# avikde/robobee3d

Measured on AMD Instinct MI355X. Metric: closed-loop MPC steps/sec (QP+dyn), higher is better.
Workload: dtype f32

## Files before the change

### robobee3d_amd/asmstep.py

```python
import functools
import os
import struct

from . import asmgen, asmtext, symbolic
from .asmgen import (A_D, A_L, A_LO, A_M, A_Q, NLDS, NVZ, S_ALPHA, S_CNT, S_ITERS, S_OMA, S_RHO, S_RINV, S_SIGMA,
                     V_W, V_WZ, V_X, V_Y, V_Z, Emit, f32bits, pk, _sb, _vp)

HERE = os.path.dirname(os.path.abspath(__file__))

PTRS = ["state", "ctrl", "ref", "ws", "out", "stats", "status", "info", "Ib", "gain", "aT0",
        "taskf", "weights", "wl", "wlu", "wlw",
        "done"]
NPTR_RES = 11
INTS = ["stride", "K", "maxIter", "nsub", "plant", "seq"]
TAIL_INTS = ["refstep"]
FLOATS = ["dt", "dtg", "Tmax", "wpr", "wpf", "ws_", "wvr", "wvf", "wds", "wthrust", "wmom",
          "iwpr", "iwpf", "iws", "iwvr", "iwvf", "iwds", "iwthrust", "iwmom",
          "Ib0", "Ib1", "Ib2", "Ibi0", "Ibi1", "Ibi2", "h", "hh", "h6", "taulim", "gpl", "idt", "mbg"]
WNAMES = ["wpr", "wpf", "ws_", "wvr", "wvf", "wds", "wthrust", "wmom"]
WROW = {"ws_": 0, "wds": 1, "wpr": 2, "wpf": 3, "wvr": 4, "wvf": 5, "wthrust": 6, "wmom": 7}
A_W, A_IW = 230, 238
S_PARAM = 4
S_PBLK = 2
S_PTR = {n: 40 + 2 * k for k, n in enumerate(PTRS[:NPTR_RES])}
S_PTR["taskf"], S_PTR["weights"] = 0, 96
S_PTR["wl"], S_PTR["wlu"], S_PTR["wlw"] = 30, 32, 34
S_INT = {"stride": 10, "K": 13, "maxIter": S_ITERS, "nsub": 5, "plant": 39}
S_F = {n: 64 + k for k, n in enumerate(FLOATS)}
assert max(S_F.values()) <= 95
S_STEP, S_SUB, S_RUIZ = 12, 15, 15
S_MBAD, S_MP0 = 62, 14
S_M0, S_M1, S_M2, S_M3 = 30, 32, 34, 36
S_C = {"minscal": 16, "maxscal": 17, "c45": 18, "eps10": 19, "eps": 38, "rho": 6, "rinv": 7, "rmin": 8,
       "rmininv": 9, "infty_ms": 100, "rhotol": 101}
S_TMP = 4
OFF = {}
_o = 0
for _n in PTRS:
    OFF[_n] = _o
    _o += 8
for _n in INTS + FLOATS + TAIL_INTS:
    OFF[_n] = _o
    _o += 4
PARAM_BYTES = _o
HIST_INTS = ["statestep", "outstep", "statusstep", "infostep"]
HIST_OFF = (PARAM_BYTES + 7) // 8 * 8
for _k, _n in enumerate(HIST_INTS):
    OFF[_n] = HIST_OFF + 4 * _k
HIST_BYTES = 4 * len(HIST_INTS)
S_HIST = 32
IMP_OFF = HIST_OFF + HIST_BYTES
assert IMP_OFF % 8 == 0
OFF["imp"], OFF["impstep"] = IMP_OFF, IMP_OFF + 8
IMP_BYTES = 16
S_IMP = 32

VFIRST, VEND = 2, 256
NRING = 6
XV_N, XV_B = 2, 254
NT_PTRS = ("state", "ctrl", "ref", "out", "stats")
A_SPARE, N_SPARE_D = 246, 9


class Pool:

    def __init__(self, e):
        self.e = e
        self.free_ = set(range(VFIRST, VEND))
        self.peak = 0
        self.fixed = set()

    def _take(self, regs):
        for r in regs:
            assert r in self.free_, "v%d is not free" % r
            self.free_.discard(r)
        self.peak = max(self.peak, VEND - VFIRST - len(self.free_))

    def reserve(self, lo, n):
        self._take(range(lo, lo + n))
        return lo

    def get(self):
        cand = sorted(self.free_)
        assert cand, "out of VGPRs"
        for r in cand:
            if (r ^ 1) not in self.free_:
                self._take([r])
                return r
        self._take([cand[0]])
        return cand[0]

    def get2(self):
        for r in sorted(self.free_):
            if r % 2 == 0 and r + 1 in self.free_:
                self._take([r, r + 1])
                return r
        raise AssertionError("out of aligned VGPR pairs")

    def get4(self):
        for r in sorted(self.free_):
            if r % 4 == 0 and all(r + k in self.free_ for k in range(4)):
                self._take([r, r + 1, r + 2, r + 3])
                return r
        raise AssertionError("out of aligned VGPR quads")

    def getn(self, n):
        for r in sorted(self.free_):
            if r % 2 == 0 and all(r + k in self.free_ for k in range(n)):
                self._take(range(r, r + n))
                return r
        raise AssertionError("out of consecutive VGPRs")

    def getn_high(self, n):
# ... 48 lines not shown
    return ("v[%d:%d]" % (base, base + 1), lo_reg % 2, hi_reg % 2)


def PS(sreg):
    if sreg % 2 == 0:
        return ("s[%d:%d]" % (sreg, sreg + 1), 0, 0)
    return ("s[%d:%d]" % (sreg - 1, sreg), 1, 1)


class Struct:
    def __init__(self, N=3, perm=None):
        s = symbolic.analyse(N, perm)
        self.s = s
        self.plan = asmgen.solve_plan(s)
        self.lpos = self.plan[2]
        self.xs, self.zs, self.xinv, self.zinv = asmgen.slot_maps(s)
        nx, nc = s.nx, s.nc
        self.neq = 2 * s.N * symbolic.NY
        self.col_of = [0] * len(s.A_i)
        self.rows = [[] for _ in range(nc)]
        for j in range(nx):
            for p in range(s.A_p[j], s.A_p[j + 1]):
                self.col_of[p] = j
                self.rows[s.A_i[p]].append(p)
        self.unit = {}
        for p, tag in enumerate(s.A_tag):
            if tag[0] == 'c' and abs(tag[1]) == 1.0 and s.A_i[p] not in self.unit:
                self.unit[s.A_i[p]] = (p, self.col_of[p])
        assert len(self.unit) == nc
        used, pairs = set(), []
        for p in range(len(s.A_i)):
            if p in used:
                continue
            i0, j0 = s.A_i[p], self.col_of[p]
            for q_ in range(p + 1, len(s.A_i)):
                if q_ in used:
                    continue
                i1, j1 = s.A_i[q_], self.col_of[q_]
                if (self.zs[i0] ^ 1) == self.zs[i1] and (j0 == j1 or (self.xs[j0] ^ 1) == self.xs[j1]):
                    lo, hi = (p, q_) if self.zs[i0] % 2 == 0 else (q_, p)
                    pairs.append((lo, hi))
                    used.update((p, q_))
                    break
        self.apairs = pairs
        self.asingles = [p for p in range(len(s.A_i)) if p not in used]
        self.apos = [0] * len(s.A_i)
        k = 0
        for (lo, hi) in pairs:
            self.apos[lo], self.apos[hi] = k, k + 1
            k += 2
        for p in self.asingles:
            self.apos[p] = k
            k += 1
        self.na = k
        self.pair_of = {}
        for (lo, hi) in pairs:
            self.pair_of[lo] = self.pair_of[hi] = (lo, hi)
        NYv = symbolic.NY
        self.qnz = list(range(s.N * NYv)) + [s.N * NYv + k_ * NYv + i for k_ in range(s.N) for i in range(3)]
        self.qslot = {}
        for j in range(s.N * NYv):
            self.qslot[j] = self.xs[j]
        base = s.N * NYv
        for k_ in range(s.N):
            for i in range(3):
                self.qslot[s.N * NYv + k_ * NYv + i] = base + 3 * k_ + i
        self.nq = base + 3 * s.N
        self.qzero = frozenset(j for j in range(nx) if j not in self.qslot)
        lnz = set(range(6)) | set(range(3 * 6, 3 * 6 + 6)) | set(range(4 * 6, 4 * 6 + 3)) | {5 * 6 + 2}
        self.lzero = frozenset(i for i in range(self.neq) if i not in lnz) if s.N == 3 else frozenset()

    def weight_of(self, j):
        N, NYv = self.s.N, symbolic.NY
        if j < N * NYv:
            k, i = divmod(j, NYv)
            return ("wpf" if k == N - 1 else "wpr") if i < 3 else "ws_"
        if j < 2 * N * NYv:
            k, i = divmod(j - N * NYv, NYv)
            return ("wvf" if k == N - 1 else "wvr") if i < 3 else "wds"
        return "wthrust" if (j - 2 * N * NYv) % 3 == 0 else "wmom"


class StepGen:
    def __init__(self, N=3, perm=None, quad=False):
        self.st = Struct(N, perm)
        self.s = self.st.s
        self.e = Emit()
        self.pool = Pool(self.e)
        self.lab = 20
        self.quad = quad
        self.nt = () if quad else ("nt",)
        self.homes = asmgen.Homes(NRING, 0 if quad else XV_N, XV_B)

    def label(self):
        self.lab += 1
        return str(self.lab)

    def rcp_nr(self, dst, src, t):
        e = self.e
        e("v_rcp_f32", v(dst), v(src))
        e("s_nop", 0)
        e("v_fma_f32", v(t), "-" + v(src), v(dst), 1.0)
        e("v_fma_f32", v(dst), v(t), v(dst), v(dst))

    def rows_ptr(self, voff, first_row):
        e = self.e
        if first_row == 0:
            e("v_mov_b32", v(voff), "v0")
        else:
            e("s_mul_i32", sg(S_TMP), sg(S_INT["stride"]), first_row)
            e("v_add_u32", v(voff), sg(S_TMP), "v0")

    def load_taskf(self):
        e = self.e
        e("s_lshl_b32", sg(S_TMP), sg(S_STEP), 5)
        e("s_load_dwordx2", sp(S_M0), sp(S_PTR["taskf"]), sg(S_TMP), "offset:0")
        e("s_load_dwordx4", "s[%d:%d]" % (S_M0 + 2, S_M0 + 5), sp(S_PTR["taskf"]), sg(S_TMP), "offset:8")
        e("s_load_dwordx2", sp(S_M0 + 6), sp(S_PTR["taskf"]), sg(S_TMP), "offset:24")
        e("s_waitcnt", "vmcnt(0) lgkmcnt(0)")

    def adv(self, voff):
        self.e("v_add_u32", v(voff), sg(S_INT["stride"]), v(voff))

    def advance_ptr(self, ptr, sstep):
        e, lo = self.e, S_PTR[ptr]
        e("s_add_i32", sg(lo), sg(lo), sg(sstep))
        e("s_cmp_lt_u32", sg(lo), sg(sstep))
        e("s_cselect_b32", sg(sstep), 1, 0)
        e("s_add_i32", sg(lo + 1), sg(lo + 1), sg(sstep))

    def impulse(self, Y0, YS):
        e = self.e
        lab_off = self.label()
        lo, hi, st, oh = S_IMP, S_IMP + 1, S_IMP + 2, S_IMP + 3
        e("s_mov_b32", sg(S_TMP), IMP_OFF)
        e("s_load_dwordx4", "s[%d:%d]" % (S_IMP, S_IMP + 3), sp(S_PBLK), sg(S_TMP))
        e("s_waitcnt", "lgkmcnt(0)")
        e("s_cmp_eq_u64", sp(lo), 0)
        e("s_cbranch_scc1", lab_off + "f")
        e("s_mul_hi_u32", sg(oh), sg(S_STEP), sg(st))
        e("s_mul_i32", sg(st), sg(S_STEP), sg(st))
        e("s_add_i32", sg(hi), sg(hi), sg(oh))
        for i in range(6):
            addend = st if i == 0 else S_INT["stride"]
            lab_nc = self.label()
            e("s_add_i32", sg(lo), sg(lo), sg(addend))
            e("s_cmp_gt_u32", sg(addend), sg(lo))
            e("s_cbranch_scc0", lab_nc + "f")
            e("s_add_i32", sg(hi), sg(hi), 1)
            e("label", lab_nc)
            e("global_load_dword", v(YS + i), "v0", sp(lo))
        e("s_waitcnt", "vmcnt(0)")
        for i in range(6):
            e("v_add_f32", v(Y0 + 12 + i), v(Y0 + 12 + i), v(YS + i))
        e("label", lab_off)

    def load_rows(self, ptr, first_row, regs, voff=None):
        own = voff is None
        if own:
            voff = self.pool.get()
        self.rows_ptr(voff, first_row)
        for k, r in enumerate(regs):
            self.e("global_load_dword", r if isinstance(r, str) else v(r), v(voff), sp(S_PTR[ptr]),
                   *(self.nt if ptr in NT_PTRS or ptr == "ws" else ()))
            if k + 1 < len(regs):
                self.adv(voff)
        if own:
            self.pool.free(voff, kill=False)

    def store_rows(self, ptr, first_row, regs, voff=None):
        own = voff is None
        if own:
            voff = self.pool.get()
        self.rows_ptr(voff, first_row)
        for k, r in enumerate(regs):
            self.e("global_store_dword", v(voff), v(r), sp(S_PTR[ptr]),
                   *(self.nt if ptr in NT_PTRS else ()))
            if k + 1 < len(regs):
                self.adv(voff)
# ... 191 lines not shown
        VP = pool.getn(nx + 1)
        VQ = pool.getn_high(st.nq + st.nq % 2)
        VA = pool.getn(st.na + st.na % 2)
        self.VP, self.VQ, self.VA = VP, VQ, VA
        RP = lambda j: VP + st.xs[j]
        RA = lambda p: VA + st.apos[p]
        RQ = lambda j: VQ + st.qslot[j]
        self.RP, self.RA, self.RQ = RP, RA, RQ
        for j in range(nx):
            e("v_accvgpr_read_b32", v(RP(j)), "a%d" % (A_W + WNAMES.index(st.weight_of(j))))
        e("v_mov_b32", v(VP + nx), 0)
        ydes = RF[0:3] + RF[6:9]
        dpdes = RF[3:6]
        WV = {n: pool.get() for n in ("wpr", "wpf", "ws_", "wvr", "wvf")}
        for n, r in WV.items():
            e("v_accvgpr_read_b32", v(r), "a%d" % (A_W + WNAMES.index(n)))
        for j in st.qnz:
            if j < N * NYv:
                k, i = divmod(j, NYv)
                wname = ("wpf" if k == N - 1 else "wpr") if i < 3 else "ws_"
                e("v_mul_f32", v(RQ(j)), "-" + v(WV[wname]), v(ydes[i]))
            else:
                k, i = divmod(j - N * NYv, NYv)
                e("v_mul_f32", v(RQ(j)), "-" + v(WV["wvf" if k == N - 1 else "wvr"]), v(dpdes[i]))
        if st.nq % 2:
            e("v_mov_b32", v(VQ + st.nq), 0)
        for p, tag in enumerate(s.A_tag):
            if tag[0] == 'c':
                e("v_mov_b32", v(RA(p)), float(tag[1]))
            elif tag[0] == 'dt':
                e("v_mov_b32", v(RA(p)), SF("dt"))
            elif tag[0] == 'T0dt':
                e("v_mov_b32", v(RA(p)), v(dtT0))
            elif tag[0] == 's0':
                e("v_mov_b32", v(RA(p)), v(s0dt[tag[1]]))
            else:
                e("v_mov_b32", v(RA(p)), v(Bdt[tag[1]]))
        if st.na % 2:
            e("v_mov_b32", v(VA + st.na), 0)
        pool.free(dtT0, *s0dt, *Bdt, t)
        pool.free(*ST)
        pool.free(*RF)
        pool.free(*WV.values())
        pool.free_range(LS, 20)
        self.ruiz_quad() if self.quad else self.ruiz()
        self.recover_and_bounds()
        self.factor()

    def maxabs(self, dst, regs, acc_in=False):
        e = self.e
        regs = list(regs)
        if not acc_in:
            if len(regs) == 1:
                e("v_and_b32", v(dst), 0x7fffffff, v(regs[0]))
                return
            if len(regs) == 2:
                e("v_max_f32", v(dst), "|%s|" % v(regs[0]), "|%s|" % v(regs[1]))
                return
            e("v_max3_f32", v(dst), "|%s|" % v(regs[0]), "|%s|" % v(regs[1]), "|%s|" % v(regs[2]))
            regs = regs[3:]
        while len(regs) >= 2:
            e("v_max3_f32", v(dst), v(dst), "|%s|" % v(regs[0]), "|%s|" % v(regs[1]))
            regs = regs[2:]
        if regs:
            e("v_max_f32", v(dst), v(dst), "|%s|" % v(regs[0]))

    def limit(self, regs, rsq):
        e = self.e
        regs = list(regs)
        prev = None
        for r in regs + [None]:
            if r is not None:
                e("v_cmp_lt_f32", "vcc", sg(S_C["minscal"]), v(r))
            if prev is not None:
                e("v_min_f32", v(prev), sg(S_C["maxscal"]), v(prev))
            if r is not None:
                e("v_cndmask_b32", v(r), 1.0, v(r), "vcc")
            prev = r
        if rsq:
            for r in regs:
                e("v_rsq_f32", v(r), v(r))
            e("s_nop", 0)

    def ruiz(self):
        e, pool, st, s = self.e, self.pool, self.st, self.s
        nx, nc = s.nx, s.nc
        RP, RA, RQ = self.RP, self.RA, self.RQ
        VE = pool.getn(nc + 1)
        self.VE = VE
        RE = lambda i: VE + st.zs[i]
        self.RE = RE
        cs = pool.get()
        self.cs = cs
        e("v_mov_b32", v(cs), 1.0)
        e("v_mov_b32", v(VE + nc), 0)
        e("s_mov_b32", sg(S_RUIZ), 10)
        top = self.label()
        e("label", top)
        for i in range(nc):
            self.maxabs(RE(i), [RA(p) for p in st.rows[i]])
        self.limit([RE(i) for i in range(nc)], rsq=True)
        colpairs = [(st.xinv[2 * k], st.xinv[2 * k + 1]) for k in range(nx // 2)]
        if nx % 2:
            colpairs.append((st.xinv[nx - 1], None))
        CH = 3
        for c0 in range(0, len(colpairs), CH):
            chunk = colpairs[c0:c0 + CH]
            T = [pool.get2() for _ in chunk]
            for (j0, j1), t2 in zip(chunk, T):
                for h, j in enumerate((j0, j1)):
                    if j is None:
                        e("v_mov_b32", v(t2 + 1), 1.0)
                        continue
                    self.maxabs(t2 + h, [RP(j)] + [RA(p) for p in range(s.A_p[j], s.A_p[j + 1])])
            self.limit([t2 + h for (j0, j1), t2 in zip(chunk, T) for h, j in enumerate((j0, j1)) if j is not None], rsq=True)
            for (j0, j1), t2 in zip(chunk, T):
                cols = [j for j in (j0, j1) if j is not None]
                tcol = {j0: t2}
                if j1 is not None:
                    tcol[j1] = t2 + 1
                ents = [p for j in cols for p in range(s.A_p[j], s.A_p[j + 1])]
                pairs = sorted({st.pair_of[p] for p in ents if p in st.pair_of})
                singles = [p for p in ents if p not in st.pair_of]
                for (lo, hi) in pairs:
                    assert st.col_of[lo] in tcol and st.col_of[hi] in tcol
                for (lo, hi) in pairs:
                    pk(e, "v_pk_mul_f32", RA(lo), [P2(RA(lo)), PSEL(RE(s.A_i[lo]), RE(s.A_i[hi]))])
                for p in singles:
                    e("v_mul_f32", v(RA(p)), v(RA(p)), v(RE(s.A_i[p])))
                if j1 is not None:
                    pk(e, "v_pk_mul_f32", RP(j0), [P2(RP(j0)), P2(t2)])
                else:
                    e("v_mul_f32", v(RP(j0)), v(RP(j0)), v(t2))
                qj = [j for j in cols if j in st.qslot]
                if len(qj) == 2 and RQ(qj[0]) % 2 == 0 and RQ(qj[1]) == RQ(qj[0]) + 1:
                    pk(e, "v_pk_mul_f32", RQ(qj[0]), [P2(RQ(qj[0])), P2(t2)])
                else:
                    for j in qj:
                        e("v_mul_f32", v(RQ(j)), v(RQ(j)), v(tcol[j]))
                for (lo, hi) in pairs:
                    pk(e, "v_pk_mul_f32", RA(lo), [P2(RA(lo)), PSEL(tcol[st.col_of[lo]], tcol[st.col_of[hi]])])
                for p in singles:
                    e("v_mul_f32", v(RA(p)), v(RA(p)), v(tcol[st.col_of[p]]))
                if j1 is not None:
                    pk(e, "v_pk_mul_f32", RP(j0), [P2(RP(j0)), P2(t2)])
                else:
                    e("v_mul_f32", v(RP(j0)), v(RP(j0)), v(t2))
            for t2 in T:
                pool.free(t2, t2 + 1)
        acc = pool.get2()
        VP, VQ = self.VP, self.VQ
        pk(e, "v_pk_add_f32", acc, [P2(VP), P2(VP + 2)])
        for k in range(4, nx + 1, 2):
            pk(e, "v_pk_add_f32", acc, [P2(acc), P2(VP + k)])
        qn, ct, t = pool.get(), pool.get(), pool.get()
        self.maxabs(qn, [VQ + k for k in range(st.nq)])
        e("v_add_f32", v(acc), v(acc), v(acc + 1))
        e("v_mul_f32", v(acc), sg(S_C["c45"]), v(acc))
        self.limit([qn], rsq=False)
        e("v_max_f32", v(acc), v(acc), v(qn))
        self.limit([acc], rsq=False)
        self.rcp_nr(ct, acc, t)
        for k in range(0, nx + 1, 2):
            pk(e, "v_pk_mul_f32", VP + k, [P2(VP + k), PB(ct)])
        for k in range(0, st.nq + st.nq % 2, 2):
            pk(e, "v_pk_mul_f32", VQ + k, [P2(VQ + k), PB(ct)])
        e("v_mul_f32", v(cs), v(cs), v(ct))
        pool.free(acc, acc + 1, qn, ct, t)
        e("s_sub_i32", sg(S_RUIZ), sg(S_RUIZ), 1)
        e("s_cmp_gt_i32", sg(S_RUIZ), 0)
        e("s_cbranch_scc1", top + "b")


    def ruiz_quad(self):
        from . import asmquad, asmquad64
        e, pool, st, s = self.e, self.pool, self.st, self.s
        nx, nc = s.nx, s.nc
        RP, RA, RQ = self.RP, self.RA, self.RQ
        VE = pool.getn(nc + 1)
        self.VE = VE
        self.RE = lambda i: VE + st.zs[i]
        cs = pool.get()
        self.cs = cs
        e("v_mov_b32", v(cs), 1.0)
        e("v_mov_b32", v(VE + nc), 0)
        qp = asmquad.QuadPlan(st)
        rp = asmquad64.RuizQuadPlan(s, qp)
        hostA = {key: RA(d[min(d)]) for key, d in rp.slots.items()}
        colmem = {}
        for j in range(nx):
            ln, C = qp.xhome[j]
            colmem.setdefault(C, {})[ln] = j
        hostP = {C: RP(m[min(m)]) for C, m in colmem.items()}
        hostQ = {C: RQ(min(jj for jj in m.values() if jj in st.qslot)) for C, m in colmem.items() if any(jj in st.qslot for jj in m.values())}
        for C, m in colmem.items():
            if C in hostQ:
                assert all(jj in st.qslot for jj in m.values())
        dead = [RA(p) for key, d in rp.slots.items() for ln, p in d.items() if RA(p) != hostA[key]] + \
               [RP(j) for C, m in colmem.items() for j in m.values() if RP(j) != hostP[C]]
        dead = sorted(set(dead))
        ET = [dead.pop() for _ in range(13)]
        DT = [dead.pop() for _ in range(15)]
        t, m7, acc, qn, ct, tt = (dead.pop() for _ in range(6))
        masks = (asmquad.S_L0, asmquad.S_L1, asmquad.S_L2)
        S_L3 = 98
        keep = sorted(set(range(self.VP, self.VP + nx + 1)) | set(range(self.VQ, self.VQ + st.nq + st.nq % 2)) |
                      set(range(self.VA, self.VA + st.na + st.na % 2)) | {cs, VE + nc})
        e("quad_begin", "ruiz")
        e("s_mov_b64", sp(asmquad.S_EXEC), "exec")
        for ln, m in enumerate(masks + (S_L3,)):
            e("s_mov_b32", sg(m), 0x11111111 << ln)
            e("s_mov_b32", sg(m + 1), 0x11111111 << ln)
            e("s_and_b64", sp(m), sp(m), sp(asmquad.S_EXEC))
        for ln in (1, 2):
            e("s_mov_b64", "exec", sp(masks[ln]))
            for key, d in rp.slots.items():
                if ln in d and RA(d[ln]) != hostA[key]:
                    e("v_mov_b32", v(hostA[key]), v(RA(d[ln])))
                elif ln not in d:
                    e("v_mov_b32", v(hostA[key]), 0)
            for C, m in colmem.items():
                if ln in m:
                    if RP(m[ln]) != hostP[C]:
                        e("v_mov_b32", v(hostP[C]), v(RP(m[ln])))
                    if C in hostQ and RQ(m[ln]) != hostQ[C]:
                        e("v_mov_b32", v(hostQ[C]), v(RQ(m[ln])))
        for key, d in rp.slots.items():
            if 0 not in d:
                e("s_mov_b64", "exec", sp(masks[0]))
                e("v_mov_b32", v(hostA[key]), 0)
                e("s_mov_b64", "exec", sp(S_L3))
                e("v_mov_b32", v(hostA[key]), 0)
        e("s_mov_b64", "exec", sp(asmquad.S_EXEC))
        e("s_nop", 4)
        e("s_mov_b32", sg(S_RUIZ), 10)
        top = self.label()
        e("label", top)
        byrow, bycol = {}, {}
        for key in sorted(rp.slots):
            byrow.setdefault(key[0], []).append(key)
            bycol.setdefault(key[1], []).append(key)
        for R in range(13):
            self.maxabs(ET[R], [hostA[k] for k in byrow[R]])
        self.limit(ET, rsq=True)
        for C in range(15):
            own = [k for k in bycol.get(C, []) if rp.kind[k] == "own"]
            self.maxabs(DT[C], [hostP[C]] + [hostA[k] for k in own])
            for k in [k for k in bycol.get(C, []) if rp.kind[k] != "own"]:
                r = hostA[k]
                e("v_max_f32_dpp", v(m7), "|%s|" % v(r), "|%s|" % v(r), asmquad.qperm(asmquad64.ROT1))
                e("v_max_f32_dpp", v(m7), "|%s|" % v(r), v(m7), asmquad.qperm(asmquad64.ROT2))
                e("s_mov_b64", "exec", sp(masks[rp.kind[k]]))
                e("v_max_f32", v(DT[C]), v(DT[C]), v(m7))
                e("s_mov_b64", "exec", sp(asmquad.S_EXEC))
                e("s_nop", 4)
# ... 1051 lines not shown
            e("s_mov_b64", "exec", sp(m))
            e("v_mov_b32", v(Q0), v(Y0 + r))
            e("v_mov_b32", v(Q0 + 1), v(Y0 + 12 + r))
            for c in range(3):
                e("v_mov_b32", v(Q0 + 2 + c), v(Y0 + 3 + r + 3 * c))
            if r == 2:
                e("v_mov_b32", v(G), SF("gpl"))
        e("s_mov_b64", "exec", sp(S_EX))
        for i in range(3):
            e("v_mov_b32", v(Q0 + 5 + i), v(Y0 + 15 + i))
        e("s_nop", 4)

        def vf(src, dst):
            p_, v_, r0, r1, r2, wx, wy, wz = (src + k for k in range(8))
            e("v_mov_b32", v(dst), v(v_))
            e("v_mul_f32", v(dst + 1), v(Th), v(r2))
            e("v_sub_f32", v(dst + 1), v(dst + 1), v(G))
            e("v_mul_f32", v(a), v(r2), v(wy))
            e("v_fma_f32", v(dst + 2), v(r1), v(wz), "-" + v(a))
            e("v_mul_f32", v(b), v(r0), v(wz))
            e("v_fma_f32", v(dst + 3), v(r2), v(wx), "-" + v(b))
            e("v_mul_f32", v(a), v(r1), v(wx))
            e("v_fma_f32", v(dst + 4), v(r0), v(wy), "-" + v(a))
            hx, hy, hz = dst + 5, dst + 6, dst + 7
            e("v_mul_f32", v(hx), v(Ib[0]), v(wx))
            e("v_mul_f32", v(hy), v(Ib[1]), v(wy))
            e("v_mul_f32", v(hz), v(Ib[2]), v(wz))
            e("v_mul_f32", v(a), v(wz), v(hy))
            e("v_fma_f32", v(a), v(wy), v(hz), "-" + v(a))
            e("v_mul_f32", v(b), v(wx), v(hz))
            e("v_fma_f32", v(b), v(wz), v(hx), "-" + v(b))
            e("v_mul_f32", v(hz), v(wy), v(hx))
            e("v_fma_f32", v(hz), v(wx), v(hy), "-" + v(hz))
            e("v_sub_f32", v(a), v(u1), v(a))
            e("v_mul_f32", v(dst + 5), v(a), v(Ibi[0]))
            e("v_sub_f32", v(b), v(u2), v(b))
            e("v_mul_f32", v(dst + 6), v(b), v(Ibi[1]))
            e("v_mul_f32", v(dst + 7), "-" + v(hz), v(Ibi[2]))
        e("s_mov_b32", sg(S_SUB), sg(S_INT["nsub"]))
        top = self.label()
        e("label", top)
        vf(Q0, QA)
        for k in range(0, 8, 2):
            pk(e, "v_pk_fma_f32", QS + k, [PS(S_F["hh"]), P2(QA + k), P2(Q0 + k)])
        vf(QS, QK)
        for k in range(0, 8, 2):
            pk(e, "v_pk_fma_f32", QA + k, [PB(two), P2(QK + k), P2(QA + k)])
            pk(e, "v_pk_fma_f32", QS + k, [PS(S_F["hh"]), P2(QK + k), P2(Q0 + k)])
        vf(QS, QK)
        for k in range(0, 8, 2):
            pk(e, "v_pk_fma_f32", QA + k, [PB(two), P2(QK + k), P2(QA + k)])
            pk(e, "v_pk_fma_f32", QS + k, [PS(S_F["h"]), P2(QK + k), P2(Q0 + k)])
        vf(QS, QK)
        for k in range(0, 8, 2):
            pk(e, "v_pk_add_f32", QA + k, [P2(QA + k), P2(QK + k)])
        for k in range(0, 8, 2):
            pk(e, "v_pk_fma_f32", Q0 + k, [PS(S_F["h6"]), P2(QA + k), P2(Q0 + k)])
        e("s_nop", 1)
        for r in range(3):
            e("v_mov_b32_dpp", v(PA + r), v(Q0), asmquad.qperm([r] * 4))
        e("s_nop", 1)
        for r in range(3):
            e("v_fmac_f32", v(serr), v(PA + r), v(PA + r))
        e("v_add_f32", v(seff), v(seff), v(einc))
        e("s_sub_i32", sg(S_SUB), sg(S_SUB), 1)
        e("s_cmp_gt_i32", sg(S_SUB), 0)
        e("s_cbranch_scc1", top + "b")
        e("s_nop", 1)
        for r in range(3):
            e("v_mov_b32_dpp", v(Y0 + r), v(Q0), asmquad.qperm([r] * 4))
            e("v_mov_b32_dpp", v(Y0 + 12 + r), v(Q0 + 1), asmquad.qperm([r] * 4))
            for c in range(3):
                e("v_mov_b32_dpp", v(Y0 + 3 + r + 3 * c), v(Q0 + 2 + c), asmquad.qperm([r] * 4))
        for i in range(3):
            e("v_mov_b32", v(Y0 + 15 + i), v(Q0 + 5 + i))
        e("s_nop", 1)
        e("quad_end", tuple(keep))

    def program(self):
        e = self.e
        self.prologue()
        top = self.label()
        e("label", top)
        self.phase_a()
        self.admm()
        self.phase_c()
        e("s_load_dword", sg(S_TMP), sp(S_PBLK), OFF["refstep"])
        e("s_load_dwordx4", "s[%d:%d]" % (S_HIST, S_HIST + 3), sp(S_PBLK), HIST_OFF)
        e("s_waitcnt", "lgkmcnt(0)")
        e("s_add_u32", sg(S_PTR["ref"]), sg(S_PTR["ref"]), sg(S_TMP))
        e("s_addc_u32", sg(S_PTR["ref"] + 1), sg(S_PTR["ref"] + 1), 0)
        for n in ("out", "status", "info"):
            self.advance_ptr(n, S_HIST + HIST_INTS.index(n + "step"))
        e("s_add_i32", sg(S_STEP), sg(S_STEP), 1)
        e("s_cmp_lt_i32", sg(S_STEP), sg(S_INT["K"]))
        e("s_cbranch_scc1", top + "b")
        e("s_waitcnt", "vmcnt(0) lgkmcnt(0)")
        lab = self.label()
        e("s_load_dwordx2", sp(S_M0), sp(S_PBLK), OFF["done"])
        e("s_load_dword", sg(S_M1), sp(S_PBLK), OFF["seq"])
        e("s_waitcnt", "lgkmcnt(0)")
        e("s_cmp_eq_u64", sp(S_M0), 0)
        e("s_cbranch_scc1", lab + "f")
        e("buffer_wbl2", "sc0 sc1")
        e("s_waitcnt", "vmcnt(0)")
        a, b = self.pool.get(), self.pool.get()
        e("v_mov_b32", v(a), 0)
        e("v_mov_b32", v(b), sg(S_M1))
        e("global_store_dword", v(a), v(b), sp(S_M0), "sc0 sc1")
        e("s_waitcnt", "vmcnt(0)")
        self.pool.free(a, b)
        e("label", lab)
        return e.ins


fmt = functools.partial(asmtext.fmt, hex_ints=asmtext.HEX_ABOVE_64)


PSEUDO = ("kill", "quad_begin", "quad_end")


def write(path=None, N=3, perm=None, quad=False):
    path = path or os.path.join(HERE, "csrc", "umpc_step_asm_quad.h" if quad else "umpc_step_asm.h")
    g = StepGen(N, perm, quad=quad)
    ins = [t for t in g.program() if t[0] not in PSEUDO]
    if quad:
        head = ["// GENERATED by robobee3d_amd/asmstep.py (quad=True) + asmquad.py -- do not edit.", asmgen.switch_banner(),
               "// The all-assembly fp32 step kernel body, ONE ROBOT PER LANE QUAD (16 robots per wavefront): %d instructions."
               % len(ins),
               "// Every lane of a quad gets the same v0 (= 4 * robot) and its own LDS slice; include umpc_step_asm.h first (StepParams).",
               "#pragma once"]
    else:
        head = ["// GENERATED by robobee3d_amd/asmstep.py -- do not edit.", asmgen.switch_banner(),
               "// The all-assembly fp32 step kernel body: %d instructions (K closed-loop steps of one wavefront)." % len(ins),
               "#pragma once", "#include <stddef.h>", "#include <stdint.h>", "namespace umpcasm {",
               "// parameter block read by the kernel with s_load (byte offsets are part of the generated code)",
               "struct StepParams {"]
        for n in PTRS:
            head.append("  const void *%s;" % n)
        for n in INTS:
            head.append("  int32_t %s;" % n)
        for n in FLOATS:
            head.append("  float %s;" % n)
        for n in TAIL_INTS:
            head.append("  int32_t %s;" % n)
        head += ["};", "static_assert(sizeof(StepParams) == %d, \"StepParams layout\");" % ((PARAM_BYTES + 7) // 8 * 8),
                "// step history (umpcBatchSetHistory): bytes the state / out / status / info pointers advance per closed-loop step,",
                "// read by the stream at byte %d of the kernarg segment: the kernels take ONE StepArgs as their first argument" % HIST_OFF,
                "struct StepHist {"] + ["  int32_t %s;" % n for n in HIST_INTS] + ["};",
                "// velocity impulses (umpcBatchSetImpulses): slice `cursor` of the table [steps][6][B] (null: none) and the bytes per slice,",
                "// read by the stream at byte %d of the kernarg segment" % IMP_OFF,
                "struct StepImp {", "  const void *imp;", "  int32_t impstep;", "  int32_t pad_;", "};",
                "struct StepArgs {", "  StepParams p;", "  StepHist h;", "  StepImp i;", "};",
                "static_assert(offsetof(StepArgs, h) == %d && sizeof(StepHist) == %d, \"StepHist layout\");" % (HIST_OFF, HIST_BYTES),
                "static_assert(offsetof(StepArgs, i) == %d && sizeof(StepImp) == %d && offsetof(StepImp, impstep) == 8, \"StepImp layout\");" % (IMP_OFF, IMP_BYTES),
                "constexpr int STEP_LDS_BYTES_PER_LANE = %d;" % (NLDS * 4), "}  // namespace umpcasm",
                "// inputs: v0 = 4 * robot, v1 = lane LDS address, s[4:5] = &StepParams (kernarg)"]
    asmtext.write_if_changed(path, asmtext.asm_block(
        head, "UMPC_STEP_ASM%s(voff, ldsaddr, params)" % ("_QUAD" if quad else ""), ins,
        '"{v0}"(voff), "{v1}"(ldsaddr), "{s[4:5]}"(params)',
        asmtext.clobbers(range(2, 256), range(256), range(4, 102)), fmt))
    return path, len(ins)


_KEEP_V = {0, 1} | set(range(V_W, V_Z)) | set(range(V_Z + 2 * 3 * symbolic.NY, V_Z + 40))
QUAD = {None: None}


def _quad():
    from . import isasim
    if QUAD[None] is None:
        QUAD.update({None: isasim.Quad(v=_KEEP_V, dead_v=set(range(256)) - _KEEP_V, a=range(A_LO, 256), dead_a=range(A_LO)),
                     "ruiz": isasim.Quad(a=range(256)), "plant": isasim.Quad(a=range(256))})
    return QUAD


FLAT = ("taskf", "wl")
STRIDE = 4096
PBASE = 0x00007E0080000000


def simulate(ins, arrays, ints, floats, max_exec=3000000, ptr_xform=None):
    import numpy as np
    from . import isasim
    base_of = {n: 0x00007F0080000000 + (k << 36) for k, n in enumerate(PTRS + ["impulse"])}
    ptr_xform = ptr_xform or (lambda a: a)
    blob = bytearray(IMP_OFF + IMP_BYTES)
    for n in PTRS:
        struct.pack_into("<Q", blob, OFF[n], ptr_xform(base_of[n]) if arrays.get(n) is not None else 0)
    allints = dict(ints, stride=STRIDE)
    allints.setdefault("seq", 0)
    allints.setdefault("refstep", 0)
    for n in HIST_INTS:
        allints.setdefault(n, 0)
    for n in INTS + TAIL_INTS + HIST_INTS:
        struct.pack_into("<i", blob, OFF[n], int(allints[n]))
    for n in FLOATS:
        struct.pack_into("<f", blob, OFF[n], float(floats[n]))
    allints.setdefault("impstep", 6 * STRIDE if arrays.get("impulse") is not None else 0)
    struct.pack_into("<Q", blob, OFF["imp"], ptr_xform(base_of["impulse"]) if arrays.get("impulse") is not None else 0)
    struct.pack_into("<i", blob, OFF["impstep"], int(allints["impstep"]))
    regions = [(PBASE, 4, np.frombuffer(bytes(blob), np.uint32))] + \
        [(base_of[n], 4 if n in FLAT else STRIDE, arrays[n]) for n in PTRS + ["impulse"] if arrays.get(n) is not None]
    m = isasim.Machine(ins, regions=regions, sgpr={S_PARAM: PBASE & 0xFFFFFFFF, S_PARAM + 1: PBASE >> 32}, vgpr={0: 0},
                       lds=np.zeros((1, NLDS), np.uint32), max_exec=max_exec, quad=_quad())
    isasim.run(m)
    simulate.last_quad_sections = {("admm" if k is None else k): n for k, n in m.sections.items()}
    simulate.last_quad_instructions = sum(m.sections.values())
    return m.nexec


if __name__ == "__main__":
    p, n = write()
    print("wrote", p, n, "instructions")


def host_floats(dt=5.0, g=9.81e-3, TtoWmax=2.0, ws=1e1, wds=1e3, wpr=1.0, wpf=5.0, wvr=1e3, wvf=2e3, wthrust=1e-1, wmom=1e-2,
                Ib=(3333.0, 3333.0, 1000.0), dtsim=0.2, taulim=100.0, mb=100.0):
    import numpy as np
    f = np.float32
    one = f(1.0)
    w = dict(wpr=f(wpr), wpf=f(wpf), ws_=f(ws), wvr=f(wvr), wvf=f(wvf), wds=f(wds), wthrust=f(wthrust), wmom=f(wmom))
    d = dict(dt=f(dt), dtg=f(f(dt) * f(g)), Tmax=f(f(TtoWmax) * f(g)), **w)
    for k, val in w.items():
        d["i" + k.rstrip("_")] = f(one / val)
    for i in range(3):
        d["Ib%d" % i] = f(Ib[i])
        d["Ibi%d" % i] = f(one / f(Ib[i]))
    d.update(h=f(dtsim), hh=f(f(0.5) * f(dtsim)), h6=f(f(dtsim) / f(6.0)), taulim=f(taulim), gpl=f(9.81e-3), idt=f(one / f(dt)),
             mbg=f(f(mb) * f(g)))
    assert set(d) == set(FLOATS), set(FLOATS) ^ set(d)
    return {k: float(val) for k, val in d.items()}
```

### robobee3d_amd/csrc/umpc_step_asm.h

```cpp
#pragma once
#include <stddef.h>
#include <stdint.h>
namespace umpcasm {
struct StepParams {
  const void *state;
  const void *ctrl;
  const void *ref;
  const void *ws;
  const void *out;
  const void *stats;
  const void *status;
  const void *info;
  const void *Ib;
  const void *gain;
  const void *aT0;
  const void *taskf;
  const void *weights;
  const void *wl;
  const void *wlu;
  const void *wlw;
  const void *done;
  int32_t stride;
  int32_t K;
  int32_t maxIter;
// ... 13 lines not shown
  float wmom;
  float iwpr;
  float iwpf;
  float iws;
  float iwvr;
  float iwvf;
  float iwds;
  float iwthrust;
  float iwmom;
  float Ib0;
  float Ib1;
  float Ib2;
  float Ibi0;
  float Ibi1;
  float Ibi2;
  float h;
  float hh;
  float h6;
  float taulim;
  float gpl;
  float idt;
  float mbg;
  int32_t refstep;
};
static_assert(sizeof(StepParams) == 296, "StepParams layout");
struct StepHist {
  int32_t statestep;
  int32_t outstep;
  int32_t statusstep;
  int32_t infostep;
};
struct StepImp {
  const void *imp;
  int32_t impstep;
  int32_t pad_;
};
struct StepArgs {
  StepParams p;
  StepHist h;
  StepImp i;
};
static_assert(offsetof(StepArgs, h) == 296 && sizeof(StepHist) == 16, "StepHist layout");
static_assert(offsetof(StepArgs, i) == 312 && sizeof(StepImp) == 16 && offsetof(StepImp, impstep) == 8, "StepImp layout");
constexpr int STEP_LDS_BYTES_PER_LANE = 640;
}
#define UMPC_STEP_ASM(voff, ldsaddr, params) asm volatile( \
  "s_mov_b64 s[2:3], s[4:5]\n" \
  "s_load_dwordx16 s[40:55], s[2:3], 0x0\n" \
  "s_load_dwordx4 s[56:59], s[2:3], 0x40\n" \
  "s_load_dwordx2 s[60:61], s[2:3], 0x50\n" \
  "s_load_dwordx2 s[0:1], s[2:3], 0x58\n" \
  "s_load_dwordx2 s[96:97], s[2:3], 0x60\n" \
  "s_load_dwordx16 s[64:79], s[2:3], 0xa0\n" \
  "s_load_dwordx16 s[80:95], s[2:3], 0xe0\n" \
  "s_load_dword s10, s[2:3], 0x88\n" \
  "s_load_dword s13, s[2:3], 0x8c\n" \
  "s_load_dword s11, s[2:3], 0x90\n" \
  "s_load_dword s5, s[2:3], 0x94\n" \
  "s_load_dword s39, s[2:3], 0x98\n" \
  "s_mov_b32 s20, 0x3fcccccd\n" \
  "s_mov_b32 s21, 0x3fcccccd\n" \
  "s_mov_b32 s22, 0xbf19999a\n" \
  "s_mov_b32 s23, 0xbf19999a\n" \
  "s_mov_b32 s24, 0x358637bd\n" \
  "s_mov_b32 s25, 0x358637bd\n" \
  "s_mov_b32 s26, 0x3c23d70a\n" \
  "s_mov_b32 s27, 0x3c23d70a\n" \
  "s_mov_b32 s28, 0x42c80000\n" \
  "s_mov_b32 s29, 0x42c80000\n" \
  "s_mov_b32 s16, 0x38d1b717\n" \
  "s_mov_b32 s17, 0x461c4000\n" \
  "s_mov_b32 s18, 0x3cb60b61\n" \
  "s_mov_b32 s38, 0x38d1b717\n" \
  "s_mov_b32 s19, 0x3a83126e\n" \
  "s_mov_b32 s6, 0x3dcccccd\n" \
  "s_mov_b32 s7, 0x41200000\n" \
  "s_mov_b32 s8, 0x358637bd\n" \
  "s_mov_b32 s9, 0x49742400\n" \
  "s_mov_b32 s100, 0x6aa56fa6\n" \
  "s_mov_b32 s101, 0x38d1b717\n" \
  "s_waitcnt lgkmcnt(0)\n" \
  "s_mov_b32 s12, 0\n" \
  "21:\n" \
  "v_mov_b32 v33, v0\n" \
  "global_load_dword v2, v33, s[40:41] nt\n" \
  "v_add_u32 v33, s10, v33\n" \
  "global_load_dword v3, v33, s[40:41] nt\n" \
  "v_add_u32 v33, s10, v33\n" \
  "global_load_dword v4, v33, s[40:41] nt\n" \
  "v_add_u32 v33, s10, v33\n" \
  "global_load_dword v5, v33, s[40:41] nt\n" \
  "v_add_u32 v33, s10, v33\n" \
  "global_load_dword v6, v33, s[40:41] nt\n" \
  "v_add_u32 v33, s10, v33\n" \
  "global_load_dword v7, v33, s[40:41] nt\n" \
  "v_add_u32 v33, s10, v33\n" \
  "global_load_dword v8, v33, s[40:41] nt\n" \
  "v_add_u32 v33, s10, v33\n" \
  "global_load_dword v9, v33, s[40:41] nt\n" \
  "v_add_u32 v33, s10, v33\n" \
  "global_load_dword v10, v33, s[40:41] nt\n" \
  "v_add_u32 v33, s10, v33\n" \
  "global_load_dword v11, v33, s[40:41] nt\n" \
  "v_add_u32 v33, s10, v33\n" \
  "global_load_dword v12, v33, s[40:41] nt\n" \
  "v_add_u32 v33, s10, v33\n" \
  "global_load_dword v13, v33, s[40:41] nt\n" \
  "v_add_u32 v33, s10, v33\n" \
  "global_load_dword v14, v33, s[40:41] nt\n" \
  "v_add_u32 v33, s10, v33\n" \
  "global_load_dword v15, v33, s[40:41] nt\n" \
  "v_add_u32 v33, s10, v33\n" \
  "global_load_dword v16, v33, s[40:41] nt\n" \
  "v_add_u32 v33, s10, v33\n" \
  "global_load_dword v17, v33, s[40:41] nt\n" \
  "v_add_u32 v33, s10, v33\n" \
  "global_load_dword v18, v33, s[40:41] nt\n" \
  "v_add_u32 v33, s10, v33\n" \
  "global_load_dword v19, v33, s[40:41] nt\n" \
  "v_mov_b32 v33, v0\n" \
  "global_load_dword v20, v33, s[44:45] nt\n" \
  "v_add_u32 v33, s10, v33\n" \
  "global_load_dword v21, v33, s[44:45] nt\n" \
  "v_add_u32 v33, s10, v33\n" \
  "global_load_dword v22, v33, s[44:45] nt\n" \
  "v_add_u32 v33, s10, v33\n" \
  "global_load_dword v23, v33, s[44:45] nt\n" \
  "v_add_u32 v33, s10, v33\n" \
  "global_load_dword v24, v33, s[44:45] nt\n" \
  "v_add_u32 v33, s10, v33\n" \
  "global_load_dword v25, v33, s[44:45] nt\n" \
  "v_add_u32 v33, s10, v33\n" \
  "global_load_dword v26, v33, s[44:45] nt\n" \
  "v_add_u32 v33, s10, v33\n" \
  "global_load_dword v27, v33, s[44:45] nt\n" \
  "v_add_u32 v33, s10, v33\n" \
  "global_load_dword v28, v33, s[44:45] nt\n" \
  "s_mul_i32 s4, s10, 0x7b\n" \
  "v_add_u32 v33, s4, v0\n" \
  "global_load_dword v29, v33, s[42:43] nt\n" \
  "v_add_u32 v33, s10, v33\n" \
  "global_load_dword v30, v33, s[42:43] nt\n" \
  "v_add_u32 v33, s10, v33\n" \
  "global_load_dword v31, v33, s[42:43] nt\n" \
  "v_add_u32 v33, s10, v33\n" \
  "global_load_dword v32, v33, s[42:43] nt\n" \
  "s_cmp_eq_u64 s[96:97], 0\n" \
  "s_cbranch_scc1 22f\n" \
  "v_mov_b32 v33, v0\n" \
  "global_load_dword v36, v33, s[96:97]\n" \
  "v_add_u32 v33, s10, v33\n" \
  "global_load_dword v39, v33, s[96:97]\n" \
  "v_add_u32 v33, s10, v33\n" \
  "global_load_dword v34, v33, s[96:97]\n" \
  "v_add_u32 v33, s10, v33\n" \
  "global_load_dword v35, v33, s[96:97]\n" \
  "v_add_u32 v33, s10, v33\n" \
  "global_load_dword v37, v33, s[96:97]\n" \
  "v_add_u32 v33, s10, v33\n" \
  "global_load_dword v38, v33, s[96:97]\n" \
  "v_add_u32 v33, s10, v33\n" \
  "global_load_dword v40, v33, s[96:97]\n" \
  "v_add_u32 v33, s10, v33\n" \
  "global_load_dword v41, v33, s[96:97]\n" \
  "s_waitcnt vmcnt(0)\n" \
  "v_rcp_f32 v42, v34\n" \
// ... 356 lines not shown
  "v_mov_b32 v145, -1.0\n" \
  "v_mov_b32 v148, s64\n" \
  "v_mov_b32 v150, -1.0\n" \
  "v_mov_b32 v152, 1.0\n" \
  "v_mov_b32 v149, s64\n" \
  "v_mov_b32 v151, -1.0\n" \
  "v_mov_b32 v153, 1.0\n" \
  "v_mov_b32 v154, s64\n" \
  "v_mov_b32 v156, -1.0\n" \
  "v_mov_b32 v158, 1.0\n" \
  "v_mov_b32 v160, s64\n" \
  "v_mov_b32 v162, -1.0\n" \
  "v_mov_b32 v164, 1.0\n" \
  "v_mov_b32 v161, s64\n" \
  "v_mov_b32 v163, -1.0\n" \
  "v_mov_b32 v165, 1.0\n" \
  "v_mov_b32 v155, s64\n" \
  "v_mov_b32 v157, -1.0\n" \
  "v_mov_b32 v159, 1.0\n" \
  "v_mov_b32 v166, s64\n" \
  "v_mov_b32 v168, -1.0\n" \
  "v_mov_b32 v170, 1.0\n" \
  "v_mov_b32 v167, s64\n" \
  "v_mov_b32 v169, -1.0\n" \
  "v_mov_b32 v171, 1.0\n" \
  "v_mov_b32 v172, s64\n" \
  "v_mov_b32 v174, -1.0\n" \
  "v_mov_b32 v176, 1.0\n" \
  "v_mov_b32 v178, s64\n" \
  "v_mov_b32 v180, -1.0\n" \
  "v_mov_b32 v182, 1.0\n" \
  "v_mov_b32 v179, s64\n" \
  "v_mov_b32 v181, -1.0\n" \
  "v_mov_b32 v183, 1.0\n" \
  "v_mov_b32 v173, s64\n" \
  "v_mov_b32 v175, -1.0\n" \
  "v_mov_b32 v177, 1.0\n" \
  "v_mov_b32 v184, s64\n" \
  "v_mov_b32 v186, -1.0\n" \
  "v_mov_b32 v185, s64\n" \
  "v_mov_b32 v187, -1.0\n" \
  "v_mov_b32 v188, s64\n" \
  "v_mov_b32 v190, -1.0\n" \
  "v_mov_b32 v192, s64\n" \
  "v_mov_b32 v194, -1.0\n" \
  "v_mov_b32 v193, s64\n" \
  "v_mov_b32 v195, -1.0\n" \
  "v_mov_b32 v189, s64\n" \
  "v_mov_b32 v191, -1.0\n" \
  "v_mov_b32 v196, v45\n" \
  "v_mov_b32 v197, v30\n" \
  "v_mov_b32 v198, v31\n" \
  "v_mov_b32 v219, 1.0\n" \
  "v_mov_b32 v200, v34\n" \
  "v_mov_b32 v201, v35\n" \
  "v_mov_b32 v199, v66\n" \
  "v_mov_b32 v202, v67\n" \
  "v_mov_b32 v203, v68\n" \
  "v_mov_b32 v220, v69\n" \
  "v_mov_b32 v204, v45\n" \
  "v_mov_b32 v205, v30\n" \
  "v_mov_b32 v221, v31\n" \
  "v_mov_b32 v222, 1.0\n" \
  "v_mov_b32 v206, v34\n" \
  "v_mov_b32 v207, v35\n" \
  "v_mov_b32 v223, v66\n" \
  "v_mov_b32 v208, v67\n" \
  "v_mov_b32 v209, v68\n" \
  "v_mov_b32 v224, v69\n" \
  "v_mov_b32 v210, v45\n" \
  "v_mov_b32 v211, v30\n" \
  "v_mov_b32 v212, v31\n" \
  "v_mov_b32 v225, 1.0\n" \
  "v_mov_b32 v214, v34\n" \
  "v_mov_b32 v215, v35\n" \
  "v_mov_b32 v213, v66\n" \
  "v_mov_b32 v216, v67\n" \
  "v_mov_b32 v217, v68\n" \
  "v_mov_b32 v226, v69\n" \
  "v_mov_b32 v227, 0\n" \
  "v_mov_b32 v42, 1.0\n" \
  "v_mov_b32 v41, 0\n" \
  "s_mov_b32 s15, 10\n" \
  "28:\n" \
  "v_max_f32 v2, |v116|, |v148|\n" \
  "v_max_f32 v3, |v117|, |v149|\n" \
  "v_max_f32 v4, |v120|, |v154|\n" \
  "v_max_f32 v6, |v124|, |v160|\n" \
  "v_max_f32 v7, |v125|, |v161|\n" \
  "v_max_f32 v5, |v121|, |v155|\n" \
  "v_max3_f32 v8, |v118|, |v130|, |v166|\n" \
  "v_max3_f32 v9, |v119|, |v131|, |v167|\n" \
  "v_max3_f32 v10, |v122|, |v134|, |v172|\n" \
  "v_max3_f32 v12, |v126|, |v138|, |v178|\n" \
  "v_max3_f32 v13, |v127|, |v139|, |v179|\n" \
  "v_max3_f32 v11, |v123|, |v135|, |v173|\n" \
  "v_max3_f32 v14, |v132|, |v142|, |v184|\n" \
  "v_max3_f32 v15, |v133|, |v143|, |v185|\n" \
  "v_max3_f32 v16, |v136|, |v144|, |v188|\n" \
  "v_max3_f32 v18, |v140|, |v146|, |v192|\n" \
  "v_max3_f32 v19, |v141|, |v147|, |v193|\n" \
  "v_max3_f32 v17, |v137|, |v145|, |v189|\n" \
  "v_max_f32 v20, |v150|, |v196|\n" \
  "v_max_f32 v21, |v151|, |v197|\n" \
  "v_max_f32 v22, |v156|, |v198|\n" \
  "v_max3_f32 v24, |v162|, |v200|, |v202|\n" \
  "v_max3_f32 v25, |v163|, |v201|, |v203|\n" \
  "v_max3_f32 v23, |v157|, |v199|, |v220|\n" \
  "v_max3_f32 v26, |v152|, |v168|, |v204|\n" \
  "v_max3_f32 v27, |v153|, |v169|, |v205|\n" \
  "v_max3_f32 v28, |v158|, |v174|, |v221|\n" \
  "v_max3_f32 v30, |v164|, |v180|, |v206|\n" \
  "v_max_f32 v30, v30, |v208|\n" \
  "v_max3_f32 v31, |v165|, |v181|, |v207|\n" \
  "v_max_f32 v31, v31, |v209|\n" \
  "v_max3_f32 v29, |v159|, |v175|, |v223|\n" \
  "v_max_f32 v29, v29, |v224|\n" \
  "v_max3_f32 v32, |v128|, |v170|, |v186|\n" \
  "v_max_f32 v32, v32, |v210|\n" \
  "v_max3_f32 v33, |v129|, |v171|, |v187|\n" \
  "v_max_f32 v33, v33, |v211|\n" \
  "v_max3_f32 v34, |v218|, |v176|, |v190|\n" \
  "v_max_f32 v34, v34, |v212|\n" \
  "v_max3_f32 v36, |v182|, |v194|, |v214|\n" \
  "v_max_f32 v36, v36, |v216|\n" \
  "v_max3_f32 v37, |v183|, |v195|, |v215|\n" \
  "v_max_f32 v37, v37, |v217|\n" \
  "v_max3_f32 v35, |v177|, |v191|, |v213|\n" \
  "v_max_f32 v35, v35, |v226|\n" \
  "v_and_b32 v38, 0x7fffffff, v219\n" \
  "v_and_b32 v39, 0x7fffffff, v222\n" \
  "v_and_b32 v40, 0x7fffffff, v225\n" \
  "v_cmp_lt_f32 vcc, s16, v2\n" \
  "v_cndmask_b32 v2, 1.0, v2, vcc\n" \
  "v_cmp_lt_f32 vcc, s16, v3\n" \
  "v_min_f32 v2, s17, v2\n" \
  "v_cndmask_b32 v3, 1.0, v3, vcc\n" \
  "v_cmp_lt_f32 vcc, s16, v4\n" \
  "v_min_f32 v3, s17, v3\n" \
  "v_cndmask_b32 v4, 1.0, v4, vcc\n" \
  "v_cmp_lt_f32 vcc, s16, v6\n" \
  "v_min_f32 v4, s17, v4\n" \
  "v_cndmask_b32 v6, 1.0, v6, vcc\n" \
  "v_cmp_lt_f32 vcc, s16, v7\n" \
  "v_min_f32 v6, s17, v6\n" \
  "v_cndmask_b32 v7, 1.0, v7, vcc\n" \
  "v_cmp_lt_f32 vcc, s16, v5\n" \
  "v_min_f32 v7, s17, v7\n" \
  "v_cndmask_b32 v5, 1.0, v5, vcc\n" \
  "v_cmp_lt_f32 vcc, s16, v8\n" \
  "v_min_f32 v5, s17, v5\n" \
  "v_cndmask_b32 v8, 1.0, v8, vcc\n" \
  "v_cmp_lt_f32 vcc, s16, v9\n" \
  "v_min_f32 v8, s17, v8\n" \
  "v_cndmask_b32 v9, 1.0, v9, vcc\n" \
  "v_cmp_lt_f32 vcc, s16, v10\n" \
  "v_min_f32 v9, s17, v9\n" \
  "v_cndmask_b32 v10, 1.0, v10, vcc\n" \
  "v_cmp_lt_f32 vcc, s16, v12\n" \
  "v_min_f32 v10, s17, v10\n" \
  "v_cndmask_b32 v12, 1.0, v12, vcc\n" \
  "v_cmp_lt_f32 vcc, s16, v13\n" \
  "v_min_f32 v12, s17, v12\n" \
  "v_cndmask_b32 v13, 1.0, v13, vcc\n" \
  "v_cmp_lt_f32 vcc, s16, v11\n" \
  "v_min_f32 v13, s17, v13\n" \
// ... 567 lines not shown
  "v_pk_add_f32 v[44:45], v[44:45], v[80:81] op_sel:[0,0] op_sel_hi:[1,1] neg_lo:[0,0] neg_hi:[0,0]\n" \
  "v_pk_add_f32 v[44:45], v[44:45], v[82:83] op_sel:[0,0] op_sel_hi:[1,1] neg_lo:[0,0] neg_hi:[0,0]\n" \
  "v_pk_add_f32 v[44:45], v[44:45], v[84:85] op_sel:[0,0] op_sel_hi:[1,1] neg_lo:[0,0] neg_hi:[0,0]\n" \
  "v_pk_add_f32 v[44:45], v[44:45], v[86:87] op_sel:[0,0] op_sel_hi:[1,1] neg_lo:[0,0] neg_hi:[0,0]\n" \
  "v_pk_add_f32 v[44:45], v[44:45], v[88:89] op_sel:[0,0] op_sel_hi:[1,1] neg_lo:[0,0] neg_hi:[0,0]\n" \
  "v_pk_add_f32 v[44:45], v[44:45], v[90:91] op_sel:[0,0] op_sel_hi:[1,1] neg_lo:[0,0] neg_hi:[0,0]\n" \
  "v_pk_add_f32 v[44:45], v[44:45], v[92:93] op_sel:[0,0] op_sel_hi:[1,1] neg_lo:[0,0] neg_hi:[0,0]\n" \
  "v_pk_add_f32 v[44:45], v[44:45], v[94:95] op_sel:[0,0] op_sel_hi:[1,1] neg_lo:[0,0] neg_hi:[0,0]\n" \
  "v_pk_add_f32 v[44:45], v[44:45], v[96:97] op_sel:[0,0] op_sel_hi:[1,1] neg_lo:[0,0] neg_hi:[0,0]\n" \
  "v_pk_add_f32 v[44:45], v[44:45], v[98:99] op_sel:[0,0] op_sel_hi:[1,1] neg_lo:[0,0] neg_hi:[0,0]\n" \
  "v_pk_add_f32 v[44:45], v[44:45], v[100:101] op_sel:[0,0] op_sel_hi:[1,1] neg_lo:[0,0] neg_hi:[0,0]\n" \
  "v_pk_add_f32 v[44:45], v[44:45], v[102:103] op_sel:[0,0] op_sel_hi:[1,1] neg_lo:[0,0] neg_hi:[0,0]\n" \
  "v_pk_add_f32 v[44:45], v[44:45], v[104:105] op_sel:[0,0] op_sel_hi:[1,1] neg_lo:[0,0] neg_hi:[0,0]\n" \
  "v_pk_add_f32 v[44:45], v[44:45], v[106:107] op_sel:[0,0] op_sel_hi:[1,1] neg_lo:[0,0] neg_hi:[0,0]\n" \
  "v_pk_add_f32 v[44:45], v[44:45], v[108:109] op_sel:[0,0] op_sel_hi:[1,1] neg_lo:[0,0] neg_hi:[0,0]\n" \
  "v_pk_add_f32 v[44:45], v[44:45], v[110:111] op_sel:[0,0] op_sel_hi:[1,1] neg_lo:[0,0] neg_hi:[0,0]\n" \
  "v_pk_add_f32 v[44:45], v[44:45], v[112:113] op_sel:[0,0] op_sel_hi:[1,1] neg_lo:[0,0] neg_hi:[0,0]\n" \
  "v_pk_add_f32 v[44:45], v[44:45], v[114:115] op_sel:[0,0] op_sel_hi:[1,1] neg_lo:[0,0] neg_hi:[0,0]\n" \
  "v_max3_f32 v43, |v228|, |v229|, |v230|\n" \
  "v_max3_f32 v43, v43, |v231|, |v232|\n" \
  "v_max3_f32 v43, v43, |v233|, |v234|\n" \
  "v_max3_f32 v43, v43, |v235|, |v236|\n" \
  "v_max3_f32 v43, v43, |v237|, |v238|\n" \
  "v_max3_f32 v43, v43, |v239|, |v240|\n" \
  "v_max3_f32 v43, v43, |v241|, |v242|\n" \
  "v_max3_f32 v43, v43, |v243|, |v244|\n" \
  "v_max3_f32 v43, v43, |v245|, |v246|\n" \
  "v_max3_f32 v43, v43, |v247|, |v248|\n" \
  "v_max3_f32 v43, v43, |v249|, |v250|\n" \
  "v_max3_f32 v43, v43, |v251|, |v252|\n" \
  "v_max3_f32 v43, v43, |v253|, |v254|\n" \
  "v_add_f32 v44, v44, v45\n" \
  "v_mul_f32 v44, s18, v44\n" \
  "v_cmp_lt_f32 vcc, s16, v43\n" \
  "v_cndmask_b32 v43, 1.0, v43, vcc\n" \
  "v_min_f32 v43, s17, v43\n" \
  "v_max_f32 v44, v44, v43\n" \
  "v_cmp_lt_f32 vcc, s16, v44\n" \
  "v_cndmask_b32 v44, 1.0, v44, vcc\n" \
  "v_min_f32 v44, s17, v44\n" \
  "v_rcp_f32 v46, v44\n" \
  "s_nop 0\n" \
  "v_fma_f32 v47, -v44, v46, 1.0\n" \
  "v_fma_f32 v46, v47, v46, v46\n" \
  "v_pk_mul_f32 v[70:71], v[70:71], v[46:47] op_sel:[0,0] op_sel_hi:[1,0] neg_lo:[0,0] neg_hi:[0,0]\n" \
  "v_pk_mul_f32 v[72:73], v[72:73], v[46:47] op_sel:[0,0] op_sel_hi:[1,0] neg_lo:[0,0] neg_hi:[0,0]\n" \
  "v_pk_mul_f32 v[74:75], v[74:75], v[46:47] op_sel:[0,0] op_sel_hi:[1,0] neg_lo:[0,0] neg_hi:[0,0]\n" \
  "v_pk_mul_f32 v[76:77], v[76:77], v[46:47] op_sel:[0,0] op_sel_hi:[1,0] neg_lo:[0,0] neg_hi:[0,0]\n" \
  "v_pk_mul_f32 v[78:79], v[78:79], v[46:47] op_sel:[0,0] op_sel_hi:[1,0] neg_lo:[0,0] neg_hi:[0,0]\n" \
  "v_pk_mul_f32 v[80:81], v[80:81], v[46:47] op_sel:[0,0] op_sel_hi:[1,0] neg_lo:[0,0] neg_hi:[0,0]\n" \
  "v_pk_mul_f32 v[82:83], v[82:83], v[46:47] op_sel:[0,0] op_sel_hi:[1,0] neg_lo:[0,0] neg_hi:[0,0]\n" \
  "v_pk_mul_f32 v[84:85], v[84:85], v[46:47] op_sel:[0,0] op_sel_hi:[1,0] neg_lo:[0,0] neg_hi:[0,0]\n" \
  "v_pk_mul_f32 v[86:87], v[86:87], v[46:47] op_sel:[0,0] op_sel_hi:[1,0] neg_lo:[0,0] neg_hi:[0,0]\n" \
  "v_pk_mul_f32 v[88:89], v[88:89], v[46:47] op_sel:[0,0] op_sel_hi:[1,0] neg_lo:[0,0] neg_hi:[0,0]\n" \
  "v_pk_mul_f32 v[90:91], v[90:91], v[46:47] op_sel:[0,0] op_sel_hi:[1,0] neg_lo:[0,0] neg_hi:[0,0]\n" \
  "v_pk_mul_f32 v[92:93], v[92:93], v[46:47] op_sel:[0,0] op_sel_hi:[1,0] neg_lo:[0,0] neg_hi:[0,0]\n" \
  "v_pk_mul_f32 v[94:95], v[94:95], v[46:47] op_sel:[0,0] op_sel_hi:[1,0] neg_lo:[0,0] neg_hi:[0,0]\n" \
  "v_pk_mul_f32 v[96:97], v[96:97], v[46:47] op_sel:[0,0] op_sel_hi:[1,0] neg_lo:[0,0] neg_hi:[0,0]\n" \
  "v_pk_mul_f32 v[98:99], v[98:99], v[46:47] op_sel:[0,0] op_sel_hi:[1,0] neg_lo:[0,0] neg_hi:[0,0]\n" \
  "v_pk_mul_f32 v[100:101], v[100:101], v[46:47] op_sel:[0,0] op_sel_hi:[1,0] neg_lo:[0,0] neg_hi:[0,0]\n" \
  "v_pk_mul_f32 v[102:103], v[102:103], v[46:47] op_sel:[0,0] op_sel_hi:[1,0] neg_lo:[0,0] neg_hi:[0,0]\n" \
  "v_pk_mul_f32 v[104:105], v[104:105], v[46:47] op_sel:[0,0] op_sel_hi:[1,0] neg_lo:[0,0] neg_hi:[0,0]\n" \
  "v_pk_mul_f32 v[106:107], v[106:107], v[46:47] op_sel:[0,0] op_sel_hi:[1,0] neg_lo:[0,0] neg_hi:[0,0]\n" \
  "v_pk_mul_f32 v[108:109], v[108:109], v[46:47] op_sel:[0,0] op_sel_hi:[1,0] neg_lo:[0,0] neg_hi:[0,0]\n" \
  "v_pk_mul_f32 v[110:111], v[110:111], v[46:47] op_sel:[0,0] op_sel_hi:[1,0] neg_lo:[0,0] neg_hi:[0,0]\n" \
  "v_pk_mul_f32 v[112:113], v[112:113], v[46:47] op_sel:[0,0] op_sel_hi:[1,0] neg_lo:[0,0] neg_hi:[0,0]\n" \
  "v_pk_mul_f32 v[114:115], v[114:115], v[46:47] op_sel:[0,0] op_sel_hi:[1,0] neg_lo:[0,0] neg_hi:[0,0]\n" \
  "v_pk_mul_f32 v[228:229], v[228:229], v[46:47] op_sel:[0,0] op_sel_hi:[1,0] neg_lo:[0,0] neg_hi:[0,0]\n" \
  "v_pk_mul_f32 v[230:231], v[230:231], v[46:47] op_sel:[0,0] op_sel_hi:[1,0] neg_lo:[0,0] neg_hi:[0,0]\n" \
  "v_pk_mul_f32 v[232:233], v[232:233], v[46:47] op_sel:[0,0] op_sel_hi:[1,0] neg_lo:[0,0] neg_hi:[0,0]\n" \
  "v_pk_mul_f32 v[234:235], v[234:235], v[46:47] op_sel:[0,0] op_sel_hi:[1,0] neg_lo:[0,0] neg_hi:[0,0]\n" \
  "v_pk_mul_f32 v[236:237], v[236:237], v[46:47] op_sel:[0,0] op_sel_hi:[1,0] neg_lo:[0,0] neg_hi:[0,0]\n" \
  "v_pk_mul_f32 v[238:239], v[238:239], v[46:47] op_sel:[0,0] op_sel_hi:[1,0] neg_lo:[0,0] neg_hi:[0,0]\n" \
  "v_pk_mul_f32 v[240:241], v[240:241], v[46:47] op_sel:[0,0] op_sel_hi:[1,0] neg_lo:[0,0] neg_hi:[0,0]\n" \
  "v_pk_mul_f32 v[242:243], v[242:243], v[46:47] op_sel:[0,0] op_sel_hi:[1,0] neg_lo:[0,0] neg_hi:[0,0]\n" \
  "v_pk_mul_f32 v[244:245], v[244:245], v[46:47] op_sel:[0,0] op_sel_hi:[1,0] neg_lo:[0,0] neg_hi:[0,0]\n" \
  "v_pk_mul_f32 v[246:247], v[246:247], v[46:47] op_sel:[0,0] op_sel_hi:[1,0] neg_lo:[0,0] neg_hi:[0,0]\n" \
  "v_pk_mul_f32 v[248:249], v[248:249], v[46:47] op_sel:[0,0] op_sel_hi:[1,0] neg_lo:[0,0] neg_hi:[0,0]\n" \
  "v_pk_mul_f32 v[250:251], v[250:251], v[46:47] op_sel:[0,0] op_sel_hi:[1,0] neg_lo:[0,0] neg_hi:[0,0]\n" \
  "v_pk_mul_f32 v[252:253], v[252:253], v[46:47] op_sel:[0,0] op_sel_hi:[1,0] neg_lo:[0,0] neg_hi:[0,0]\n" \
  "v_pk_mul_f32 v[254:255], v[254:255], v[46:47] op_sel:[0,0] op_sel_hi:[1,0] neg_lo:[0,0] neg_hi:[0,0]\n" \
  "v_mul_f32 v42, v42, v46\n" \
  "s_sub_i32 s15, s15, 1\n" \
  "s_cmp_gt_i32 s15, 0\n" \
  "s_cbranch_scc1 28b\n" \
  "v_rcp_f32 v43, v42\n" \
  "s_nop 0\n" \
  "v_fma_f32 v44, -v42, v43, 1.0\n" \
  "v_fma_f32 v43, v44, v43, v43\n" \
  "s_mul_i32 s4, s10, 9\n" \
  "v_add_u32 v47, s4, v0\n" \
  "v_accvgpr_read_b32 v48, a238\n" \
  "v_accvgpr_read_b32 v49, a239\n" \
  "v_accvgpr_read_b32 v50, a240\n" \
  "v_accvgpr_read_b32 v51, a241\n" \
  "v_accvgpr_read_b32 v52, a242\n" \
  "v_accvgpr_read_b32 v53, a243\n" \
  "v_accvgpr_read_b32 v54, a244\n" \
  "v_accvgpr_read_b32 v55, a245\n" \
  "v_mul_f32 v45, v70, v43\n" \
  "v_mul_f32 v45, v48, v45\n" \
  "v_sqrt_f32 v45, v45\n" \
  "s_nop 0\n" \
  "v_accvgpr_write_b32 a246, v45\n" \
  "v_rcp_f32 v46, v45\n" \
  "s_nop 0\n" \
  "v_mul_f32 v2, |v116|, v46\n" \
  "v_mul_f32 v8, |v118|, v46\n" \
  "v_mul_f32 v45, v71, v43\n" \
  "v_mul_f32 v45, v48, v45\n" \
  "v_sqrt_f32 v45, v45\n" \
  "s_nop 0\n" \
  "v_accvgpr_write_b32 a247, v45\n" \
  "v_rcp_f32 v46, v45\n" \
  "s_nop 0\n" \
  "v_mul_f32 v3, |v117|, v46\n" \
  "v_mul_f32 v9, |v119|, v46\n" \
  "v_mul_f32 v45, v72, v43\n" \
  "v_mul_f32 v45, v48, v45\n" \
  "v_sqrt_f32 v45, v45\n" \
  "s_nop 0\n" \
  "v_accvgpr_write_b32 a248, v45\n" \
  "v_rcp_f32 v46, v45\n" \
  "s_nop 0\n" \
  "v_mul_f32 v4, |v120|, v46\n" \
  "v_mul_f32 v10, |v122|, v46\n" \
  "v_mul_f32 v45, v74, v43\n" \
  "v_mul_f32 v45, v50, v45\n" \
  "v_sqrt_f32 v45, v45\n" \
  "s_nop 0\n" \
  "v_accvgpr_write_b32 a249, v45\n" \
  "v_rcp_f32 v46, v45\n" \
  "s_nop 0\n" \
  "v_mul_f32 v6, |v124|, v46\n" \
  "v_mul_f32 v12, |v126|, v46\n" \
  "v_mul_f32 v45, v75, v43\n" \
  "v_mul_f32 v45, v50, v45\n" \
  "v_sqrt_f32 v45, v45\n" \
  "s_nop 0\n" \
  "v_accvgpr_write_b32 a250, v45\n" \
  "v_rcp_f32 v46, v45\n" \
  "s_nop 0\n" \
  "v_mul_f32 v7, |v125|, v46\n" \
  "v_mul_f32 v13, |v127|, v46\n" \
  "v_mul_f32 v45, v73, v43\n" \
  "v_mul_f32 v45, v50, v45\n" \
  "v_sqrt_f32 v45, v45\n" \
  "s_nop 0\n" \
  "v_accvgpr_write_b32 a251, v45\n" \
  "v_rcp_f32 v46, v45\n" \
  "s_nop 0\n" \
  "v_mul_f32 v5, |v121|, v46\n" \
  "v_mul_f32 v11, |v123|, v46\n" \
  "v_mul_f32 v45, v76, v43\n" \
  "v_mul_f32 v45, v48, v45\n" \
  "v_sqrt_f32 v45, v45\n" \
  "s_nop 0\n" \
  "v_accvgpr_write_b32 a252, v45\n" \
  "v_rcp_f32 v46, v45\n" \
  "s_nop 0\n" \
  "v_mul_f32 v14, |v132|, v46\n" \
  "v_mul_f32 v45, v77, v43\n" \
  "v_mul_f32 v45, v48, v45\n" \
  "v_sqrt_f32 v45, v45\n" \
  "s_nop 0\n" \
  "v_accvgpr_write_b32 a253, v45\n" \
  "v_rcp_f32 v46, v45\n" \
  "s_nop 0\n" \
// ... 7783 lines not shown
```

### robobee3d_amd/isasim.py

```python
import functools
import re
from fractions import Fraction

import numpy as np

f32, f64, u32, u64 = np.float32, np.float64, np.uint32, np.uint64
POISON = 0x7ff8dead
VCC = 106
LANE_LDS_VGPR = 1


class AddressFault(Exception):
    """A simulated global access outside every array handed to the interpreter (on the GPU: a memory access fault)."""


class Quad:

    def __init__(self, v=(), a=(), lds=(), dead_v=(), dead_a=(), dead_lds=()):
        self.v, self.a, self.lds = list(v), list(a), list(lds)
        self.dead_v, self.dead_a, self.dead_lds = list(dead_v), list(dead_a), list(dead_lds)


_REG = re.compile(r"([vas])(\d+)$|([vas])\[(\d+):(\d+)\]$")

# ... 10 lines not shown
    x = x[1:-1] if ab else x
    if x == "vcc":
        return ("s", VCC, 2, neg, ab)
    if x == "exec":
        return ("exec", 0, 2, neg, ab)
    mm = _REG.match(x)
    if mm is None:
        raise ValueError("operand %r" % x)
    if mm.group(1):
        return (mm.group(1), int(mm.group(2)), 1, neg, ab)
    return (mm.group(3), int(mm.group(4)), int(mm.group(5)) - int(mm.group(4)) + 1, neg, ab)


@functools.lru_cache(maxsize=None)
def _regs(x):
    if not isinstance(x, str):
        return frozenset()
    x = x.lstrip("-").strip("|")
    if x == "vcc":
        return frozenset({("s", VCC), ("s", VCC + 1)})
    mm = _REG.match(x)
    if mm is None:
        return frozenset()
    if mm.group(1):
        return frozenset({(mm.group(1), int(mm.group(2)))})
    return frozenset((mm.group(3), r) for r in range(int(mm.group(4)), int(mm.group(5)) + 1))


def _srcs(t, k):
    x, d = t[k], t[-1]
    if isinstance(x, dict):
        return frozenset()
    if not isinstance(d, dict) or k < 2:
        return _regs(x)
    kind, lo = _decode(x)[:2]
    q = k - 2
    sels = (d["op_sel"][q],) if t[0] == "v_pk_mov_b32" else (d["op_sel"][q], d["op_sel_hi"][q])
    return frozenset((kind, lo + h) for h in sels)


def _fmax(a, b):
    return np.where(b != b, a, np.where(a != a, b, np.where(b > a, b, a)))


def _fmin(a, b):
    return np.where(b != b, a, np.where(a != a, b, np.where(b < a, b, a)))


def _imm(t, k):
    for x in t[k:]:
        if isinstance(x, int):
            return x
        if isinstance(x, str) and x.startswith("offset:"):
            return int(x[7:])
    return 0


_CMP = {"lt": np.less, "le": np.less_equal, "gt": np.greater, "ge": np.greater_equal, "eq": np.equal,
        "nlt": lambda a, b: ~(a < b), "neq": lambda a, b: ~(a == b), "ne": np.not_equal, "u": lambda a, b: (a != a) | (b != b)}
_WAITABLE = ("ds_read", "global_load", "s_load")
_T1_READ = ("ds_write", "ds_min", "global_store", "s_cmp", "s_cbranch", "s_branch", "v_fmac")


class Machine:
    def __init__(self, ins, lanes=1, regions=(), sgpr=None, vgpr=None, lds=None, max_exec=3000000, quad=None, log=None,
                 V=None, A=None):
        self.ins, self.lanes = ins, lanes
        self.V = np.full((lanes, 256), POISON, u32) if V is None else V
        self.A = np.full((lanes, 256), POISON, u32) if A is None else A
        self.S = [0] * 128
        for r, val in (sgpr or {}).items():
            self.S[r] = val & 0xFFFFFFFF
        if V is None:
            for r, val in (vgpr or {}).items():
                self.V[:, r] = val
            self.V[:, LANE_LDS_VGPR] = 16 * np.arange(lanes)
        self.lds = np.zeros((1, 0), u32) if lds is None else lds
        self.regions = [(b, st, arr, arr.view(u32).reshape(-1), arr.itemsize) for b, st, arr in regions]
        self.set_exec(np.ones(lanes, bool))
        self.scc = 0
        self.max_exec, self.quad, self.log = max_exec, quad or {}, log
        self.nexec = 0
        self.sections = {}
        self.pend = {"vmcnt": [], "lgkmcnt": []}
        self.labels = {}
        for k, t in enumerate(ins):
            if t[0] == "label":
                self.labels.setdefault(t[1], []).append(k)
        self._use, self._rw = {}, {}
        self.dead = set()
        self.src_word, self.src_phase, self.phase = {}, {}, 0

    def set_exec(self, bits):
        self.exec, self.full, self.any = bits, bool(bits.all()), bool(bits.any())

    def mask64(self, bits):
        return sum(1 << ln for ln in range(self.lanes) if bits[ln])

    def lanes_of(self, m):
        return np.array([(m >> ln) & 1 for ln in range(self.lanes)], bool)

    def s32(self, x):
        k, lo = _decode(x)[:2]
        return lo & 0xFFFFFFFF if k == "i" else self.S[lo]

    def s64(self, x):
        k, lo = _decode(x)[:2]
        if k == "i":
            return lo & 0xFFFFFFFFFFFFFFFF
        if k == "exec":
            return self.mask64(self.exec)
        return self.S[lo] | (self.S[lo + 1] << 32)

    def set64(self, x, val):
        k, lo = _decode(x)[:2]
        if k == "exec":
            self.set_exec(self.lanes_of(val))
        else:
            self.S[lo], self.S[lo + 1] = val & 0xFFFFFFFF, (val >> 32) & 0xFFFFFFFF

    def bits(self, x, dpp=None):
        k, lo, _, neg, ab = _decode(x)
        if k == "f":
            b = np.full(self.lanes, np.array(lo, f32).view(u32), u32)
        elif k == "i":
            b = np.full(self.lanes, lo & 0xFFFFFFFF, u32)
        elif k == "s":
            b = np.full(self.lanes, self.S[lo], u32)
        else:
            b = (self.V if k == "v" else self.A)[:, lo].copy()
            if dpp is not None:
                qp = [int(c) for c in dpp[dpp.index("[") + 1:dpp.index("]")].split(",")][:self.lanes]
                for ln in range(self.lanes):
                    if self.exec[ln] and not self.exec[qp[ln]]:
                        raise AssertionError("DPP read of a masked-off lane: %r" % (dpp,))
                b = b[qp]
        if ab:
            b = b & u32(0x7FFFFFFF)
        return b ^ u32(0x80000000) if neg else b

    def f(self, x, dpp=None):
        return self.bits(x, dpp).view(f32)

    def d(self, x):
        k, lo, _, neg, ab = _decode(x)
        if k == "f":
            val = np.full(self.lanes, lo, f64)
        else:
            if k == "s":
                b = np.full(self.lanes, self.S[lo] | (self.S[lo + 1] << 32), u64)
            else:
                R = self.V if k == "v" else self.A
                b = R[:, lo].astype(u64) | (R[:, lo + 1].astype(u64) << u64(32))
            val = b.view(f64)
        if ab:
            val = np.abs(val)
        return -val if neg else val

    def write(self, x, b, lo_off=0):
        k, lo = _decode(x)[:2]
        R = self.V if k == "v" else self.A
        if self.full:
            R[:, lo + lo_off] = b
        else:
            R[self.exec, lo + lo_off] = np.asarray(b, u32)[self.exec]

# ... 28 lines not shown
        w = (byte // 1024) * 4 + (byte % 16) // 4
        if w >= self.lds.shape[1]:
            raise AddressFault("%r touches LDS byte 0x%x, outside the lane's slice" % (self.ins[self.pc], byte))
        return ln, w

    def active(self):
        return [ln for ln in range(self.lanes) if self.exec[ln]]

    def uses(self, pc):
        u = self._use.get(pc)
        if u is None:
            t = self.ins[pc]
            u = self._use[pc] = set().union(*[_regs(x) for x in t[1:] if not isinstance(x, dict)])
        return u

    def wait(self, t):
        for part in " ".join(str(x) for x in t[1:]).split():
            name, val = part[:-1].split("(")
            del self.pend[name][:max(0, len(self.pend[name]) - int(val))]

    def track(self, pc, m):
        used = self.uses(pc)
        for q in self.pend.values():
            for dst in q:
                assert not (dst & used), ("register used before its load was waited for", pc, self.ins[pc], sorted(dst & used))
        if m.startswith(_WAITABLE):
            (self.pend["vmcnt"] if m.startswith("global") else self.pend["lgkmcnt"]).append(_regs(self.ins[pc][1]))
        elif m.startswith("ds_"):
            self.pend["lgkmcnt"].append(set())
        elif m.startswith("global_"):
            self.pend["vmcnt"].append(set())
        if self.dead:
            rw = self._rw.get(pc)
            if rw is None:
                t = self.ins[pc]
                dst = frozenset() if m.startswith(_T1_READ) else _regs(t[1])
                rw = self._rw[pc] = (set().union(*[_srcs(t, k) for k in range(2 if dst else 1, len(t))]), dst)
            assert not (rw[0] & self.dead), ("register read after its kill", pc, self.ins[pc], sorted(rw[0] & self.dead))
            self.dead -= rw[1]
        if self.log is not None:
            self.log_reads(pc, m, used)

    def log_reads(self, pc, m, used):
        if m.startswith("ds_read"):
            return
        t = self.ins[pc]
        wr_only = _regs(t[1]) if m in ("global_load_dword", "v_mov_b32", "v_accvgpr_read_b32") else set()
        for r in wr_only:
            self.src_word.pop(r, None)
        for r in used - wr_only:
            if r in self.src_word:
                if self.src_phase[r] == self.phase:
                    self.log["r"].add(self.src_word[r])
                else:
                    self.log["late"].add((self.src_phase[r], self.src_word[r]))

    def branch(self, target):
        lab, d = target[:-1], target[-1]
        cands = self.labels[lab]
        self.pc = min(c for c in cands if c > self.pc) if d == "f" else max(c for c in cands if c < self.pc)

    def run(self, pc=0):
        ins = self.ins
        self.pc = pc
        with np.errstate(all="ignore"):
            while self.pc < len(ins):
                t = ins[self.pc]
                m = t[0]
                if m == "label":
                    self.pc += 1
                    continue
                if m == "kill":
                    self.V[:, _decode(t[1])[1]] = POISON
                    self.dead |= _regs(t[1])
                    self.pc += 1
                    continue
                if m == "quad_begin":
                    self.run_quad(t)
                    continue
                if m == "quad_end":
                    return
                self.nexec += 1
                assert self.nexec < self.max_exec, "runaway program"
                if m == "s_waitcnt":
                    self.wait(t)
                elif m == "s_barrier":
                    assert not self.pend["lgkmcnt"], ("s_barrier with LDS operations in flight: another wave may not see them", self.pc)
                    yield self.pc
                    self.phase += 1
                else:
                    op = OPS.get(m)
                    if op is None:
                        raise ValueError("unknown instruction %r" % (t,))
                    self.track(self.pc, m)
                    if self.any or m in SALU or m == "v_readfirstlane_b32":
                        op(self, t)
                self.pc += 1

    def run_quad(self, t):
        assert self.lanes == 1 and self.exec.all()
        name = t[1] if len(t) > 1 else None
        spec = self.quad[name]
        q = Machine(self.ins, 4, lds=np.tile(self.lds, (4, 1)), max_exec=self.max_exec,
                    V=np.tile(self.V, (4, 1)), A=np.tile(self.A, (4, 1)))
        q.V[:, LANE_LDS_VGPR] += 16 * np.arange(4, dtype=u32)
        q.S, q.scc, q.regions, q.pend, q.labels, q._use = self.S, self.scc, self.regions, self.pend, self.labels, self._use
        for _ in q.run(self.pc + 1):
            raise AssertionError("s_barrier inside a quad section")
        end = self.ins[q.pc]
        assert q.exec.all() and not any(dst for pend in self.pend.values() for dst in pend), \
            ("EXEC not restored / loads outstanding at the end of the quad section", name)
        q.V[:, LANE_LDS_VGPR] -= 16 * np.arange(4, dtype=u32)
        outs_v = spec.v + (list(end[1]) if len(end) > 1 else [])
        for R, R4, outs, dead in ((self.V, q.V, outs_v, spec.dead_v), (self.A, q.A, spec.a, spec.dead_a),
                                  (self.lds, q.lds, spec.lds, spec.dead_lds)):
            agree = (R4[1:] == R4[0]).all(0)
            bad = [r for r in outs if not agree[r]]
            assert not bad, "lanes of the quad disagree on %r after the %s section" % (bad[:8], name or "quad")
            R[0] = np.where(agree, R4[0], u32(POISON))
            R[0, dead] = POISON
        self.sections[name] = self.sections.get(name, 0) + q.nexec
        self.nexec += q.nexec
        self.scc = q.scc
        self.pc = q.pc + 1


def run(m):
    for _ in m.run():
        pass
    return m.nexec


def run_group(machines):
    nw = len(machines)
    logs = []
    for mc in machines:
        mc.log = dict(r=set(), w=set(), a=set(), late=set())
        logs.append(mc.log)
    gens = [mc.run() for mc in machines]
    live = [True] * nw
    nbar = 0
    hist = []
    while any(live):
        for w in range(nw):
            if live[w]:
                try:
                    next(gens[w])
                except StopIteration:
                    live[w] = False
        assert all(live) or not any(live), ("the waves disagree about barrier %d" % nbar, live)
        for a_ in range(nw):
            for b_ in range(nw):
                if a_ != b_:
                    clash = (logs[a_]["w"] & (logs[b_]["r"] | logs[b_]["w"] | logs[b_]["a"])) | (logs[a_]["a"] & logs[b_]["r"])
                    assert not clash, ("LDS race before barrier %d: words written by wave %d and touched by wave %d" % (nbar, a_, b_),
                                       sorted(clash)[:8], {k_: sorted(clash & v_)[:4] for k_, v_ in logs[b_].items() if k_ != "late"})
        hist.append([lg["w"] | lg["a"] for lg in logs])
        for b_ in range(nw):
            for (ph, word) in logs[b_]["late"]:
                for a_ in range(nw):
                    assert a_ == b_ or ph >= len(hist) or word not in hist[ph][a_], \
                        ("LDS race: word %d fetched by wave %d in phase %d (looked at later) was written by wave %d in that phase" % (word, b_, ph, a_))
        for lg in logs:
            for st_ in lg.values():
                st_.clear()
        nbar += 1
# ... 27 lines not shown
    return f


def _s_and_saveexec(mc, t):
    old = mc.mask64(mc.exec)
    mc.set64(t[1], old)
    mc.set_exec(mc.lanes_of(old & mc.s64(t[2])))
    mc.scc = int(mc.exec.any())


def _s_load(mc, t):
    n = 1 if t[0] == "s_load_dword" else int(t[0][len("s_load_dwordx"):])
    words, w0 = mc.gaddr(t[2], None, mc.s32(t[3]) + _imm(t, 4), 0, n)
    lo = _decode(t[1])[1]
    for k in range(n):
        mc.S[lo + k] = int(words[w0 + k])


def _cbranch(cond):
    def f(mc, t):
        if cond(mc):
            mc.branch(t[1])
    return f


def _nop(mc, t):
    pass


SALU = {
    "s_nop": _nop, "buffer_wbl2": _nop,
    "s_mov_b32": lambda mc, t: _sdst(mc, t, mc.s32(t[2])),
    "s_mov_b64": _s_mov_b64,
    "s_mul_i32": lambda mc, t: _sdst(mc, t, mc.s32(t[2]) * mc.s32(t[3])),
    "s_mul_hi_u32": lambda mc, t: _sdst(mc, t, (mc.s32(t[2]) * mc.s32(t[3])) >> 32),
    "s_add_u32": _s_add,
    "s_addc_u32": lambda mc, t: _s_add(mc, t, mc.scc),
    "s_add_i32": lambda mc, t: _sdst(mc, t, mc.s32(t[2]) + mc.s32(t[3])),
    "s_sub_i32": lambda mc, t: _sdst(mc, t, mc.s32(t[2]) - mc.s32(t[3])),
    "s_lshl_b32": lambda mc, t: _sdst(mc, t, mc.s32(t[2]) << (mc.s32(t[3]) & 31)),
    "s_cmp_lt_i32": lambda mc, t: setattr(mc, "scc", int(_signed(mc.s32(t[1])) < _signed(mc.s32(t[2])))),
    "s_cmp_gt_i32": lambda mc, t: setattr(mc, "scc", int(_signed(mc.s32(t[1])) > _signed(mc.s32(t[2])))),
    "s_cmp_lt_u32": lambda mc, t: setattr(mc, "scc", int(mc.s32(t[1]) < mc.s32(t[2]))),
    "s_cmp_gt_u32": lambda mc, t: setattr(mc, "scc", int(mc.s32(t[1]) > mc.s32(t[2]))),
    "s_cselect_b32": lambda mc, t: _sdst(mc, t, mc.s32(t[2]) if mc.scc else mc.s32(t[3])),
    "s_cmp_lg_u32": lambda mc, t: setattr(mc, "scc", int(mc.s32(t[1]) != mc.s32(t[2]))),
    "s_cmp_eq_u32": lambda mc, t: setattr(mc, "scc", int(mc.s32(t[1]) == mc.s32(t[2]))),
    "s_cmp_eq_u64": lambda mc, t: setattr(mc, "scc", int(mc.s64(t[1]) == mc.s64(t[2]))),
    "s_and_b64": _s_logic(lambda a, b: a & b),
    "s_or_b64": _s_logic(lambda a, b: a | b),
    "s_andn2_b64": _s_logic(lambda a, b: a & ~b),
    "s_and_saveexec_b64": _s_and_saveexec,
    "s_branch": _cbranch(lambda mc: True),
    "s_cbranch_scc1": _cbranch(lambda mc: mc.scc),
    "s_cbranch_scc0": _cbranch(lambda mc: not mc.scc),
    "s_cbranch_vccz": _cbranch(lambda mc: (mc.S[VCC] | mc.S[VCC + 1]) == 0),
    "s_cbranch_vccnz": _cbranch(lambda mc: (mc.S[VCC] | mc.S[VCC + 1]) != 0),
    "s_cbranch_execz": _cbranch(lambda mc: not mc.exec.any()),
}
for _n in (1, 2, 4, 8, 16):
    SALU["s_load_dword" + ("x%d" % _n if _n > 1 else "")] = _s_load


def _f32op(op, dpp=False):
    def f(mc, t):
        srcs = t[2:-1] if dpp else t[2:]
        vals = [mc.f(srcs[0], t[-1] if dpp else None)] + [mc.f(x) for x in srcs[1:]]
        mc.wf(t[1], op(*vals))
    return f


def _fma32(a, b, c):
    return (a.astype(f64) * b.astype(f64) + c.astype(f64)).astype(f32)


def _fmac(dpp=False):
    def f(mc, t):
        a = mc.f(t[2], t[4] if dpp else None)
        mc.wf(t[1], _fma32(a, mc.f(t[3]), mc.f(t[1])))
    return f


def _nanless(red):
    def f(a, b, c):
        out = np.empty_like(a)
        for ln in range(len(a)):
            vals = [x for x in (a[ln], b[ln], c[ln]) if x == x]
            out[ln] = red(vals) if vals else f32(np.nan)
        return out
    return f


def _f64op(op):
    def f(mc, t):
        mc.wd(t[1], op(*[mc.d(x) for x in t[2:]]))
    return f


def _fma64(a, b, c):
    out = a * b + c
    for ln in range(len(a)):
        if np.isfinite(a[ln]) and np.isfinite(b[ln]) and np.isfinite(c[ln]):
            out[ln] = float(Fraction(float(a[ln])) * Fraction(float(b[ln])) + Fraction(float(c[ln])))
    return out


def _pk(kind):
    def f(mc, t):
        d = t[-1]
        srcs = t[2:-1]
        res = []
        for hi in (0, 1):
            sel = d["op_sel_hi"] if hi else d["op_sel"]
            ng = d["neg_hi"] if hi else d["neg_lo"]
            vals = [mc.half(x, sel[q]) * (-1 if ng[q] else 1) for q, x in enumerate(srcs)]
            if kind == "fma":
                res.append((vals[0] * vals[1] + vals[2]).astype(f32))
            elif kind == "mul":
                res.append(vals[0].astype(f32) * vals[1].astype(f32))
            else:
                res.append(vals[0].astype(f32) + vals[1].astype(f32))
        for h in (0, 1):
            mc.write(t[1], res[h].view(u32), h)
    return f


def _pk_mov(mc, t):
    sel = t[-1]["op_sel"]
    halves = [mc.bits("%s%d" % (x[0], _decode(x)[1] + sel[q])) for q, x in enumerate(t[2:4])]
    mc.write(t[1], halves[0])
    mc.write(t[1], halves[1], 1)


def _cmp(kind):
    def f(mc, t):
        op = _CMP[t[0][len("v_cmp_"):].split("_")[0]]
        if kind == "f32":
            cond = op(mc.f(t[2]), mc.f(t[3]))
        elif kind == "f64":
            cond = op(mc.d(t[2]), mc.d(t[3]))
        else:
            cond = op(mc.bits(t[2]), mc.bits(t[3]))
        mc.wmask(t[1], np.asarray(cond, bool))
    return f


def _cndmask(mc, t):
    sel = mc.lanes_of(mc.s64(t[4] if len(t) > 4 else "vcc"))
    mc.write(t[1], np.where(sel, mc.bits(t[3]), mc.bits(t[2])).astype(u32))


def _ds(mc, t):
    m = t[0]
    n = {"b32": 1, "b64": 2, "b128": 4, "f32": 1}[m.rsplit("_", 1)[1]]
    read = m.startswith("ds_read")
    base, reg = (t[2], t[1]) if read else (t[1], t[2])
    k, lo = _decode(reg)[:2]
    for ln in mc.active():
        sl, w = mc.lds_word(base, t[3], ln)
        if read:
            mc.V[ln, lo:lo + n] = mc.lds[sl, w:w + n]
        elif m == "ds_min_f32":
            cur, val = mc.lds[sl, w:w + 1].view(f32)[0], mc.V[ln, lo:lo + 1].view(f32)[0]
            mc.lds[sl, w] = np.array(val if val < cur else cur, f32).view(u32)
        else:
            mc.lds[sl, w:w + n] = mc.V[ln, lo:lo + n]
    if mc.log is not None:
        sl, w = mc.lds_word(base, t[3], mc.active()[0])
        if read:
            for h in range(n):
                mc.src_word[("v", lo + h)], mc.src_phase[("v", lo + h)] = w + h, mc.phase
        else:
            mc.log["a" if m == "ds_min_f32" else "w"].update(range(w, w + n))


def _global(mc, t):
    m = t[0]
    n = {"dword": 1, "dwordx2": 2, "dwordx4": 4}[m.rsplit("_", 1)[1]]
    load = m.startswith("global_load")
    voff, reg = (t[2], t[1]) if load else (t[1], t[2])
    k, lo = _decode(reg)[:2]
    R = mc.V if k == "v" else mc.A
    for ln in mc.active():
        words, w0 = mc.gaddr(t[3], voff, _imm(t, 4), ln, n)
        if load:
            R[ln, lo:lo + n] = words[w0:w0 + n]
        else:
            words[w0:w0 + n] = R[ln, lo:lo + n]


def _readfirstlane(mc, t):
    act = mc.active()
    mc.S[_decode(t[1])[1]] = int(mc.bits(t[2])[act[0] if act else 0])


def _bitop(op):
    return lambda mc, t: mc.write(t[1], op(mc.bits(t[2]).astype(u64), mc.bits(t[3]).astype(u64)).astype(u32))


VECTOR = {
    "v_mov_b32": lambda mc, t: mc.write(t[1], mc.bits(t[2])),
    "v_mov_b32_dpp": lambda mc, t: mc.write(t[1], mc.bits(t[2], t[3])),
    "v_accvgpr_read_b32": lambda mc, t: mc.write(t[1], mc.bits(t[2])),
    "v_accvgpr_write_b32": lambda mc, t: mc.write(t[1], mc.bits(t[2])),
    "v_readfirstlane_b32": _readfirstlane,
    "v_pk_mov_b32": _pk_mov,
    "v_add_u32": _bitop(lambda a, b: (a + b) & u64(0xFFFFFFFF)),
    "v_and_b32": _bitop(lambda a, b: a & b),
    "v_or_b32": _bitop(lambda a, b: a | b),
    "v_lshrrev_b32": _bitop(lambda a, b: b >> (a & u64(31))),
    "v_mul_u32_u24": _bitop(lambda a, b: ((a & u64(0xFFFFFF)) * (b & u64(0xFFFFFF))) & u64(0xFFFFFFFF)),
    "v_bfe_u32": lambda mc, t: mc.write(t[1], (mc.bits(t[2]) >> u32(t[3] & 31)) & u32((1 << t[4]) - 1)),
    "v_cvt_f32_i32": lambda mc, t: mc.wf(t[1], mc.bits(t[2]).view(np.int32).astype(f32)),
    "v_fma_f32": _f32op(_fma32),
    "v_fmac_f32": _fmac(),
    "v_fmac_f32_dpp": _fmac(True),
    "v_fmaak_f32": lambda mc, t: mc.wf(t[1], _fma32(mc.f(t[2]), mc.f(t[3]), mc.f(t[4]))),
    "v_mul_f32": _f32op(lambda a, b: a * b),
    "v_mul_f32_dpp": _f32op(lambda a, b: a * b, True),
    "v_add_f32": _f32op(lambda a, b: a + b),
    "v_add_f32_dpp": _f32op(lambda a, b: a + b, True),
    "v_sub_f32": _f32op(lambda a, b: a - b),
    "v_subrev_f32": _f32op(lambda a, b: b - a),
    "v_max_f32": _f32op(_fmax),
    "v_max_f32_dpp": _f32op(_fmax, True),
    "v_min_f32": _f32op(_fmin),
    "v_max3_f32": _f32op(_nanless(max)),
    "v_min3_f32": _f32op(_nanless(min)),
    "v_med3_f32": _f32op(lambda a, b, c: np.sort(np.stack([a, b, c]), 0)[1]),
    "v_rcp_f32": _f32op(lambda a: f32(1.0) / a),
    "v_rsq_f32": _f32op(lambda a: (1.0 / np.sqrt(a.astype(f64))).astype(f32)),
    "v_sqrt_f32": _f32op(lambda a: np.sqrt(a.astype(f64)).astype(f32)),
    "v_pk_fma_f32": _pk("fma"),
    "v_pk_mul_f32": _pk("mul"),
    "v_pk_add_f32": _pk("add"),
    "v_cndmask_b32": _cndmask,
    "v_cndmask_b32_e64": _cndmask,
    "v_fma_f64": _f64op(_fma64),
    "v_mul_f64": _f64op(lambda a, b: a * b),
    "v_add_f64": _f64op(lambda a, b: a + b),
    "v_max_f64": _f64op(_fmax),
    "v_min_f64": _f64op(_fmin),
    "v_rcp_f64": _f64op(lambda a: 1.0 / a),
    "v_rsq_f64": _f64op(lambda a: 1.0 / np.sqrt(a)),
    "v_cmp_nlt_f64": _cmp("f64"),
    "v_cmp_eq_i32_e64": _cmp("int"),
    "v_cmp_ne_u32": _cmp("int"),
}
for _op in ("lt", "le", "gt", "ge", "eq", "nlt", "neq", "u"):
    VECTOR["v_cmp_%s_f32" % _op] = VECTOR["v_cmp_%s_f32_e64" % _op] = _cmp("f32")
OPS = dict(SALU, **VECTOR)
for _m in ("ds_read_b32", "ds_read_b64", "ds_read_b128", "ds_write_b32", "ds_write_b64", "ds_write_b128", "ds_min_f32",
           "global_load_dword", "global_load_dwordx2", "global_load_dwordx4", "global_store_dword", "global_store_dwordx2"):
    OPS[_m] = _ds if _m.startswith("ds_") else _global
```

Before: 539.1 million.

## Speculatively skip Ruiz scaling clamps, restart exactly if bounds are violated

The Ruiz equilibration loop now runs a speculative variant by default. It drops the per-scaling min/max clamp (compare, cndmask, min) and instead tracks a running min and max of all scalings. After the loop, if any tracked value fell outside [minscal, maxscal], or if a finite-check on the inputs found a NaN, the step restarts from the top in exact mode. This cuts VALU work in the hot equilibration loop, at the cost of extra tracking instructions, a larger code footprint, and a full recompute of the step whenever the clamp would have been needed.

```diff
diff --git a/robobee3d_amd/asmstep.py b/robobee3d_amd/asmstep.py
--- a/robobee3d_amd/asmstep.py
+++ b/robobee3d_amd/asmstep.py
@@ -29,6 +29,7 @@
 S_F = {n: 64 + k for k, n in enumerate(FLOATS)}
 assert max(S_F.values()) <= 95
 S_STEP, S_SUB, S_RUIZ = 12, 15, 15
+S_EXACT = 14
 S_MBAD, S_MP0 = 62, 14
 S_M0, S_M1, S_M2, S_M3 = 30, 32, 34, 36
 S_C = {"minscal": 16, "maxscal": 17, "c45": 18, "eps10": 19, "eps": 38, "rho": 6, "rinv": 7, "rmin": 8,
@@ -243,19 +244,26 @@
 
 
 class StepGen:
-    def __init__(self, N=3, perm=None, quad=False):
+    def __init__(self, N=3, perm=None, quad=False, exact_ruiz=False):
         self.st = Struct(N, perm)
         self.s = self.st.s
         self.e = Emit()
         self.pool = Pool(self.e)
         self.lab = 20
+        self.lab_spec = 500
         self.quad = quad
+        self.speculate = not quad and not exact_ruiz
+        self.ruiz_span = self.restart_at = None
         self.nt = () if quad else ("nt",)
         self.homes = asmgen.Homes(NRING, 0 if quad else XV_N, XV_B)
 
     def label(self):
         self.lab += 1
         return str(self.lab)
+
+    def label_spec(self):
+        self.lab_spec += 1
+        return str(self.lab_spec)
 
     def rcp_nr(self, dst, src, t):
         e = self.e
@@ -613,24 +621,107 @@
                 e("v_rsq_f32", v(r), v(r))
             e("s_nop", 0)
 
+    def scalings(self, regs, track):
+        if track is None:
+            return self.limit(regs, rsq=True)
+        e = self.e
+        regs = list(regs)
+        lo, hi = track
+        for k in range(0, len(regs) - 1, 2):
+            e("v_min3_f32", v(lo), v(lo), v(regs[k]), v(regs[k + 1]))
+            e("v_max3_f32", v(hi), v(hi), v(regs[k]), v(regs[k + 1]))
+        if len(regs) % 2:
+            e("v_min_f32", v(lo), v(lo), v(regs[-1]))
+            e("v_max_f32", v(hi), v(hi), v(regs[-1]))
+        for r in regs:
+            e("v_rsq_f32", v(r), v(r))
+        e("s_nop", 0)
+
     def ruiz(self):
         e, pool, st, s = self.e, self.pool, self.st, self.s
-        nx, nc = s.nx, s.nc
-        RP, RA, RQ = self.RP, self.RA, self.RQ
+        nc = s.nc
         VE = pool.getn(nc + 1)
         self.VE = VE
-        RE = lambda i: VE + st.zs[i]
-        self.RE = RE
+        self.RE = lambda i: VE + st.zs[i]
         cs = pool.get()
         self.cs = cs
         e("v_mov_b32", v(cs), 1.0)
         e("v_mov_b32", v(VE + nc), 0)
         e("s_mov_b32", sg(S_RUIZ), 10)
-        top = self.label()
-        e("label", top)
+        first = len(e.ins)
+        if not self.speculate:
+            top = self.label()
+            e("label", top)
+            self.ruiz_pass(None)
+            e("s_sub_i32", sg(S_RUIZ), sg(S_RUIZ), 1)
+            e("s_cmp_gt_i32", sg(S_RUIZ), 0)
+            e("s_cbranch_scc1", top + "b")
+            self.ruiz_span = (first, len(e.ins))
+            return
+        self.finite_guard()
+        lab_x = self.label()
+        lab_f, lab_more, lab_done = (self.label_spec() for _ in range(3))
+        e("label", lab_x)
+        self.ruiz_pass(None)
+        e("s_sub_i32", sg(S_RUIZ), sg(S_RUIZ), 1)
+        e("s_cmp_lg_u32", sg(S_EXACT), 0)
+        e("s_cbranch_scc1", lab_more + "f")
+        track = (pool.get(), pool.get())
+        for r in track:
+            e("v_mov_b32", v(r), 1.0)
+        e("label", lab_f)
+        self.ruiz_pass(track)
+        e("s_sub_i32", sg(S_RUIZ), sg(S_RUIZ), 1)
+        e("s_cmp_gt_i32", sg(S_RUIZ), 0)
+        e("s_cbranch_scc1", lab_f + "b")
+        e("v_cmp_lt_f32_e64", sp(S_M0), sg(S_C["minscal"]), v(track[0]))
+        e("v_cmp_ge_f32_e64", sp(S_M1), sg(S_C["maxscal"]), v(track[1]))
+        e("s_and_b64", sp(S_M0), sp(S_M0), sp(S_M1))
+        e("s_andn2_b64", sp(S_M0), "exec", sp(S_M0))
+        e("s_cbranch_scc0", lab_done + "f")
+        e("s_mov_b32", sg(S_EXACT), 1)
+        e("s_waitcnt", "vmcnt(0) lgkmcnt(0)")
+        self.restart_at = len(e.ins)
+        e("s_branch", self.lab_restart + "b")
+        e("label", lab_more)
+        e("s_cmp_gt_i32", sg(S_RUIZ), 0)
+        e("s_cbranch_scc1", lab_x + "b")
+        e("label", lab_done)
+        pool.free(*track)
+        self.ruiz_span = (first, len(e.ins))
+
+    def finite_guard(self):
+        e, pool, st, s = self.e, self.pool, self.st, self.s
+        zero = PB(self.VE + s.nc)
+        acc = pool.get2()
+        nq2 = st.nq + st.nq % 2
+        pk(e, "v_pk_mul_f32", acc, [zero, P2(self.VQ)])
+        for k in range(2, nq2, 2):
+            pk(e, "v_pk_fma_f32", acc, [zero, P2(self.VQ + k), P2(acc)])
+        reps = {}
+        for p_, tag in enumerate(s.A_tag):
+            if tag[0] != 'c':
+                reps.setdefault(tag[0] if tag[0] in ("dt", "T0dt") else tuple(tag[:2]), self.RA(p_))
+        for j in range(s.nx):
+            reps.setdefault(st.weight_of(j), self.RP(j))
+        assert len(reps) == 11 + len(WNAMES)
+        for r in reps.values():
+            e("v_fma_f32", v(acc), 0, v(r), v(acc))
+        lab = self.label_spec()
+        e("v_cmp_u_f32", "vcc", v(acc), v(acc + 1))
+        e("s_cmp_eq_u64", "vcc", 0)
+        e("s_cbranch_scc1", lab + "f")
+        e("s_mov_b32", sg(S_EXACT), 1)
+        e("label", lab)
+        pool.free(acc, acc + 1)
+
+    def ruiz_pass(self, track):
+        e, pool, st, s = self.e, self.pool, self.st, self.s
+        nx, nc = s.nx, s.nc
+        RP, RA, RQ, RE, cs = self.RP, self.RA, self.RQ, self.RE, self.cs
         for i in range(nc):
             self.maxabs(RE(i), [RA(p) for p in st.rows[i]])
-        self.limit([RE(i) for i in range(nc)], rsq=True)
+        self.scalings([RE(i) for i in range(nc)], track)
         colpairs = [(st.xinv[2 * k], st.xinv[2 * k + 1]) for k in range(nx // 2)]
         if nx % 2:
             colpairs.append((st.xinv[nx - 1], None))
@@ -644,7 +735,7 @@
                         e("v_mov_b32", v(t2 + 1), 1.0)
                         continue
                     self.maxabs(t2 + h, [RP(j)] + [RA(p) for p in range(s.A_p[j], s.A_p[j + 1])])
-            self.limit([t2 + h for (j0, j1), t2 in zip(chunk, T) for h, j in enumerate((j0, j1)) if j is not None], rsq=True)
+            self.scalings([t2 + h for (j0, j1), t2 in zip(chunk, T) for h, j in enumerate((j0, j1)) if j is not None], track)
             for (j0, j1), t2 in zip(chunk, T):
                 cols = [j for j in (j0, j1) if j is not None]
                 tcol = {j0: t2}
@@ -698,10 +789,6 @@
             pk(e, "v_pk_mul_f32", VQ + k, [P2(VQ + k), PB(ct)])
         e("v_mul_f32", v(cs), v(cs), v(ct))
         pool.free(acc, acc + 1, qn, ct, t)
-        e("s_sub_i32", sg(S_RUIZ), sg(S_RUIZ), 1)
-        e("s_cmp_gt_i32", sg(S_RUIZ), 0)
-        e("s_cbranch_scc1", top + "b")
-
 
     def ruiz_quad(self):
         from . import asmquad, asmquad64
@@ -1919,6 +2006,10 @@
         self.prologue()
         top = self.label()
         e("label", top)
+        if self.speculate:
+            e("s_mov_b32", sg(S_EXACT), 0)
+            self.lab_restart = self.label_spec()
+            e("label", self.lab_restart)
         self.phase_a()
         self.admm()
         self.phase_c()
@@ -2017,7 +2108,7 @@
 PBASE = 0x00007E0080000000
 
 
-def simulate(ins, arrays, ints, floats, max_exec=3000000, ptr_xform=None):
+def simulate(ins, arrays, ints, floats, max_exec=3000000, ptr_xform=None, lanes=1, hits=False):
     import numpy as np
     from . import isasim
     base_of = {n: 0x00007F0080000000 + (k << 36) for k, n in enumerate(PTRS + ["impulse"])}
@@ -2025,7 +2116,8 @@
     blob = bytearray(IMP_OFF + IMP_BYTES)
     for n in PTRS:
         struct.pack_into("<Q", blob, OFF[n], ptr_xform(base_of[n]) if arrays.get(n) is not None else 0)
-    allints = dict(ints, stride=STRIDE)
+    stride = STRIDE if lanes == 1 else 4 * lanes
+    allints = dict(ints, stride=stride)
     allints.setdefault("seq", 0)
     allints.setdefault("refstep", 0)
     for n in HIST_INTS:
@@ -2034,14 +2126,20 @@
         struct.pack_into("<i", blob, OFF[n], int(allints[n]))
     for n in FLOATS:
         struct.pack_into("<f", blob, OFF[n], float(floats[n]))
-    allints.setdefault("impstep", 6 * STRIDE if arrays.get("impulse") is not None else 0)
+    allints.setdefault("impstep", 6 * stride if arrays.get("impulse") is not None else 0)
     struct.pack_into("<Q", blob, OFF["imp"], ptr_xform(base_of["impulse"]) if arrays.get("impulse") is not None else 0)
     struct.pack_into("<i", blob, OFF["impstep"], int(allints["impstep"]))
     regions = [(PBASE, 4, np.frombuffer(bytes(blob), np.uint32))] + \
-        [(base_of[n], 4 if n in FLAT else STRIDE, arrays[n]) for n in PTRS + ["impulse"] if arrays.get(n) is not None]
-    m = isasim.Machine(ins, regions=regions, sgpr={S_PARAM: PBASE & 0xFFFFFFFF, S_PARAM + 1: PBASE >> 32}, vgpr={0: 0},
-                       lds=np.zeros((1, NLDS), np.uint32), max_exec=max_exec, quad=_quad())
+        [(base_of[n], 4 if n in FLAT or lanes > 1 else STRIDE, arrays[n].reshape(-1))
+         for n in PTRS + ["impulse"] if arrays.get(n) is not None]
+    assert all(arrays[n].flags.c_contiguous for n in PTRS + ["impulse"] if arrays.get(n) is not None)
+    m = isasim.Machine(ins, lanes, regions=regions, sgpr={S_PARAM: PBASE & 0xFFFFFFFF, S_PARAM + 1: PBASE >> 32},
+                       vgpr={0: 4 * np.arange(lanes)}, lds=np.zeros((lanes, NLDS), np.uint32), max_exec=max_exec,
+                       quad=_quad() if lanes == 1 else None)
+    if hits:
+        m.hits = np.zeros(len(ins), np.int64)
     isasim.run(m)
+    simulate.last_hits = m.hits
     simulate.last_quad_sections = {("admm" if k is None else k): n for k, n in m.sections.items()}
     simulate.last_quad_instructions = sum(m.sections.values())
     return m.nexec
diff --git a/robobee3d_amd/csrc/umpc_step_asm.h b/robobee3d_amd/csrc/umpc_step_asm.h
--- a/robobee3d_amd/csrc/umpc_step_asm.h
+++ b/robobee3d_amd/csrc/umpc_step_asm.h
@@ -119,6 +119,8 @@
   "s_waitcnt lgkmcnt(0)\n" \
   "s_mov_b32 s12, 0\n" \
   "21:\n" \
+  "s_mov_b32 s14, 0\n" \
+  "501:\n" \
   "v_mov_b32 v33, v0\n" \
   "global_load_dword v2, v33, s[40:41] nt\n" \
   "v_add_u32 v33, s10, v33\n" \
@@ -641,6 +643,44 @@
   "v_mov_b32 v42, 1.0\n" \
   "v_mov_b32 v41, 0\n" \
   "s_mov_b32 s15, 10\n" \
+  "v_pk_mul_f32 v[44:45], v[40:41], v[228:229] op_sel:[1,0] op_sel_hi:[1,1] neg_lo:[0,0] neg_hi:[0,0]\n" \
+  "v_pk_fma_f32 v[44:45], v[40:41], v[230:231], v[44:45] op_sel:[1,0,0] op_sel_hi:[1,1,1] neg_lo:[0,0,0] neg_hi:[0,0,0]\n" \
+  "v_pk_fma_f32 v[44:45], v[40:41], v[232:233], v[44:45] op_sel:[1,0,0] op_sel_hi:[1,1,1] neg_lo:[0,0,0] neg_hi:[0,0,0]\n" \
+  "v_pk_fma_f32 v[44:45], v[40:41], v[234:235], v[44:45] op_sel:[1,0,0] op_sel_hi:[1,1,1] neg_lo:[0,0,0] neg_hi:[0,0,0]\n" \
+  "v_pk_fma_f32 v[44:45], v[40:41], v[236:237], v[44:45] op_sel:[1,0,0] op_sel_hi:[1,1,1] neg_lo:[0,0,0] neg_hi:[0,0,0]\n" \
+  "v_pk_fma_f32 v[44:45], v[40:41], v[238:239], v[44:45] op_sel:[1,0,0] op_sel_hi:[1,1,1] neg_lo:[0,0,0] neg_hi:[0,0,0]\n" \
+  "v_pk_fma_f32 v[44:45], v[40:41], v[240:241], v[44:45] op_sel:[1,0,0] op_sel_hi:[1,1,1] neg_lo:[0,0,0] neg_hi:[0,0,0]\n" \
+  "v_pk_fma_f32 v[44:45], v[40:41], v[242:243], v[44:45] op_sel:[1,0,0] op_sel_hi:[1,1,1] neg_lo:[0,0,0] neg_hi:[0,0,0]\n" \
+  "v_pk_fma_f32 v[44:45], v[40:41], v[244:245], v[44:45] op_sel:[1,0,0] op_sel_hi:[1,1,1] neg_lo:[0,0,0] neg_hi:[0,0,0]\n" \
+  "v_pk_fma_f32 v[44:45], v[40:41], v[246:247], v[44:45] op_sel:[1,0,0] op_sel_hi:[1,1,1] neg_lo:[0,0,0] neg_hi:[0,0,0]\n" \
+  "v_pk_fma_f32 v[44:45], v[40:41], v[248:249], v[44:45] op_sel:[1,0,0] op_sel_hi:[1,1,1] neg_lo:[0,0,0] neg_hi:[0,0,0]\n" \
+  "v_pk_fma_f32 v[44:45], v[40:41], v[250:251], v[44:45] op_sel:[1,0,0] op_sel_hi:[1,1,1] neg_lo:[0,0,0] neg_hi:[0,0,0]\n" \
+  "v_pk_fma_f32 v[44:45], v[40:41], v[252:253], v[44:45] op_sel:[1,0,0] op_sel_hi:[1,1,1] neg_lo:[0,0,0] neg_hi:[0,0,0]\n" \
+  "v_pk_fma_f32 v[44:45], v[40:41], v[254:255], v[44:45] op_sel:[1,0,0] op_sel_hi:[1,1,1] neg_lo:[0,0,0] neg_hi:[0,0,0]\n" \
+  "v_fma_f32 v44, 0, v128, v44\n" \
+  "v_fma_f32 v44, 0, v148, v44\n" \
+  "v_fma_f32 v44, 0, v196, v44\n" \
+  "v_fma_f32 v44, 0, v197, v44\n" \
+  "v_fma_f32 v44, 0, v198, v44\n" \
+  "v_fma_f32 v44, 0, v200, v44\n" \
+  "v_fma_f32 v44, 0, v201, v44\n" \
+  "v_fma_f32 v44, 0, v199, v44\n" \
+  "v_fma_f32 v44, 0, v202, v44\n" \
+  "v_fma_f32 v44, 0, v203, v44\n" \
+  "v_fma_f32 v44, 0, v220, v44\n" \
+  "v_fma_f32 v44, 0, v70, v44\n" \
+  "v_fma_f32 v44, 0, v74, v44\n" \
+  "v_fma_f32 v44, 0, v82, v44\n" \
+  "v_fma_f32 v44, 0, v88, v44\n" \
+  "v_fma_f32 v44, 0, v92, v44\n" \
+  "v_fma_f32 v44, 0, v100, v44\n" \
+  "v_fma_f32 v44, 0, v106, v44\n" \
+  "v_fma_f32 v44, 0, v107, v44\n" \
+  "v_cmp_u_f32 vcc, v44, v45\n" \
+  "s_cmp_eq_u64 vcc, 0\n" \
+  "s_cbranch_scc1 502f\n" \
+  "s_mov_b32 s14, 1\n" \
+  "502:\n" \
   "28:\n" \
   "v_max_f32 v2, |v116|, |v148|\n" \
   "v_max_f32 v3, |v117|, |v149|\n" \
@@ -1374,8 +1414,591 @@
   "v_pk_mul_f32 v[254:255], v[254:255], v[46:47] op_sel:[0,0] op_sel_hi:[1,0] neg_lo:[0,0] neg_hi:[0,0]\n" \
   "v_mul_f32 v42, v42, v46\n" \
   "s_sub_i32 s15, s15, 1\n" \
+  "s_cmp_lg_u32 s14, 0\n" \
+  "s_cbranch_scc1 504f\n" \
+  "v_mov_b32 v43, 1.0\n" \
+  "v_mov_b32 v44, 1.0\n" \
+  "503:\n" \
+  "v_max_f32 v2, |v116|, |v148|\n" \
+  "v_max_f32 v3, |v117|, |v149|\n" \
+  "v_max_f32 v4, |v120|, |v154|\n" \
+  "v_max_f32 v6, |v124|, |v160|\n" \
+  "v_max_f32 v7, |v125|, |v161|\n" \
+  "v_max_f32 v5, |v121|, |v155|\n" \
+  "v_max3_f32 v8, |v118|, |v130|, |v166|\n" \
+  "v_max3_f32 v9, |v119|, |v131|, |v167|\n" \
+  "v_max3_f32 v10, |v122|, |v134|, |v172|\n" \
+  "v_max3_f32 v12, |v126|, |v138|, |v178|\n" \
+  "v_max3_f32 v13, |v127|, |v139|, |v179|\n" \
+  "v_max3_f32 v11, |v123|, |v135|, |v173|\n" \
+  "v_max3_f32 v14, |v132|, |v142|, |v184|\n" \
+  "v_max3_f32 v15, |v133|, |v143|, |v185|\n" \
+  "v_max3_f32 v16, |v136|, |v144|, |v188|\n" \
+  "v_max3_f32 v18, |v140|, |v146|, |v192|\n" \
+  "v_max3_f32 v19, |v141|, |v147|, |v193|\n" \
+  "v_max3_f32 v17, |v137|, |v145|, |v189|\n" \
+  "v_max_f32 v20, |v150|, |v196|\n" \
+  "v_max_f32 v21, |v151|, |v197|\n" \
+  "v_max_f32 v22, |v156|, |v198|\n" \
+  "v_max3_f32 v24, |v162|, |v200|, |v202|\n" \
+  "v_max3_f32 v25, |v163|, |v201|, |v203|\n" \
+  "v_max3_f32 v23, |v157|, |v199|, |v220|\n" \
+  "v_max3_f32 v26, |v152|, |v168|, |v204|\n" \
+  "v_max3_f32 v27, |v153|, |v169|, |v205|\n" \
+  "v_max3_f32 v28, |v158|, |v174|, |v221|\n" \
+  "v_max3_f32 v30, |v164|, |v180|, |v206|\n" \
+  "v_max_f32 v30, v30, |v208|\n" \
+  "v_max3_f32 v31, |v165|, |v181|, |v207|\n" \
+  "v_max_f32 v31, v31, |v209|\n" \
+  "v_max3_f32 v29, |v159|, |v175|, |v223|\n" \
+  "v_max_f32 v29, v29, |v224|\n" \
+  "v_max3_f32 v32, |v128|, |v170|, |v186|\n" \
+  "v_max_f32 v32, v32, |v210|\n" \
+  "v_max3_f32 v33, |v129|, |v171|, |v187|\n" \
+  "v_max_f32 v33, v33, |v211|\n" \
+  "v_max3_f32 v34, |v218|, |v176|, |v190|\n" \
+  "v_max_f32 v34, v34, |v212|\n" \
+  "v_max3_f32 v36, |v182|, |v194|, |v214|\n" \
+  "v_max_f32 v36, v36, |v216|\n" \
+  "v_max3_f32 v37, |v183|, |v195|, |v215|\n" \
+  "v_max_f32 v37, v37, |v217|\n" \
+  "v_max3_f32 v35, |v177|, |v191|, |v213|\n" \
+  "v_max_f32 v35, v35, |v226|\n" \
+  "v_and_b32 v38, 0x7fffffff, v219\n" \
+  "v_and_b32 v39, 0x7fffffff, v222\n" \
+  "v_and_b32 v40, 0x7fffffff, v225\n" \
+  "v_min3_f32 v43, v43, v2, v3\n" \
+  "v_max3_f32 v44, v44, v2, v3\n" \
+  "v_min3_f32 v43, v43, v4, v6\n" \
+  "v_max3_f32 v44, v44, v4, v6\n" \
+  "v_min3_f32 v43, v43, v7, v5\n" \
+  "v_max3_f32 v44, v44, v7, v5\n" \
+  "v_min3_f32 v43, v43, v8, v9\n" \
+  "v_max3_f32 v44, v44, v8, v9\n" \
+  "v_min3_f32 v43, v43, v10, v12\n" \
+  "v_max3_f32 v44, v44, v10, v12\n" \
+  "v_min3_f32 v43, v43, v13, v11\n" \
+  "v_max3_f32 v44, v44, v13, v11\n" \
+  "v_min3_f32 v43, v43, v14, v15\n" \
+  "v_max3_f32 v44, v44, v14, v15\n" \
+  "v_min3_f32 v43, v43, v16, v18\n" \
+  "v_max3_f32 v44, v44, v16, v18\n" \
+  "v_min3_f32 v43, v43, v19, v17\n" \
+  "v_max3_f32 v44, v44, v19, v17\n" \
+  "v_min3_f32 v43, v43, v20, v21\n" \
+  "v_max3_f32 v44, v44, v20, v21\n" \
+  "v_min3_f32 v43, v43, v22, v24\n" \
+  "v_max3_f32 v44, v44, v22, v24\n" \
+  "v_min3_f32 v43, v43, v25, v23\n" \
+  "v_max3_f32 v44, v44, v25, v23\n" \
+  "v_min3_f32 v43, v43, v26, v27\n" \
+  "v_max3_f32 v44, v44, v26, v27\n" \
+  "v_min3_f32 v43, v43, v28, v30\n" \
+  "v_max3_f32 v44, v44, v28, v30\n" \
+  "v_min3_f32 v43, v43, v31, v29\n" \
+  "v_max3_f32 v44, v44, v31, v29\n" \
+  "v_min3_f32 v43, v43, v32, v33\n" \
+  "v_max3_f32 v44, v44, v32, v33\n" \
+  "v_min3_f32 v43, v43, v34, v36\n" \
+  "v_max3_f32 v44, v44, v34, v36\n" \
+  "v_min3_f32 v43, v43, v37, v35\n" \
+  "v_max3_f32 v44, v44, v37, v35\n" \
+  "v_min3_f32 v43, v43, v38, v39\n" \
+  "v_max3_f32 v44, v44, v38, v39\n" \
+  "v_min_f32 v43, v43, v40\n" \
+  "v_max_f32 v44, v44, v40\n" \
+  "v_rsq_f32 v2, v2\n" \
+  "v_rsq_f32 v3, v3\n" \
+  "v_rsq_f32 v4, v4\n" \
+  "v_rsq_f32 v6, v6\n" \
+  "v_rsq_f32 v7, v7\n" \
+  "v_rsq_f32 v5, v5\n" \
+  "v_rsq_f32 v8, v8\n" \
+  "v_rsq_f32 v9, v9\n" \
+  "v_rsq_f32 v10, v10\n" \
+  "v_rsq_f32 v12, v12\n" \
+  "v_rsq_f32 v13, v13\n" \
+  "v_rsq_f32 v11, v11\n" \
+  "v_rsq_f32 v14, v14\n" \
+  "v_rsq_f32 v15, v15\n" \
+  "v_rsq_f32 v16, v16\n" \
+  "v_rsq_f32 v18, v18\n" \
+  "v_rsq_f32 v19, v19\n" \
+  "v_rsq_f32 v17, v17\n" \
+  "v_rsq_f32 v20, v20\n" \
+  "v_rsq_f32 v21, v21\n" \
+  "v_rsq_f32 v22, v22\n" \
+  "v_rsq_f32 v24, v24\n" \
+  "v_rsq_f32 v25, v25\n" \
+  "v_rsq_f32 v23, v23\n" \
+  "v_rsq_f32 v26, v26\n" \
+  "v_rsq_f32 v27, v27\n" \
+  "v_rsq_f32 v28, v28\n" \
+  "v_rsq_f32 v30, v30\n" \
+  "v_rsq_f32 v31, v31\n" \
+  "v_rsq_f32 v29, v29\n" \
+  "v_rsq_f32 v32, v32\n" \
+  "v_rsq_f32 v33, v33\n" \
+  "v_rsq_f32 v34, v34\n" \
+  "v_rsq_f32 v36, v36\n" \
+  "v_rsq_f32 v37, v37\n" \
+  "v_rsq_f32 v35, v35\n" \
+  "v_rsq_f32 v38, v38\n" \
+  "v_rsq_f32 v39, v39\n" \
+  "v_rsq_f32 v40, v40\n" \
+  "s_nop 0\n" \
+  "v_max3_f32 v46, |v70|, |v116|, |v118|\n" \
+  "v_max3_f32 v47, |v71|, |v117|, |v119|\n" \
+  "v_max3_f32 v48, |v72|, |v120|, |v122|\n" \
+  "v_max3_f32 v49, |v73|, |v121|, |v123|\n" \
+  "v_max_f32 v49, v49, |v218|\n" \
+  "v_max3_f32 v50, |v74|, |v124|, |v126|\n" \
+  "v_max_f32 v50, v50, |v128|\n" \
+  "v_max3_f32 v51, |v75|, |v125|, |v127|\n" \
+  "v_max_f32 v51, v51, |v129|\n" \
+  "v_min3_f32 v43, v43, v46, v47\n" \
+  "v_max3_f32 v44, v44, v46, v47\n" \
+  "v_min3_f32 v43, v43, v48, v49\n" \
+  "v_max3_f32 v44, v44, v48, v49\n" \
+  "v_min3_f32 v43, v43, v50, v51\n" \
+  "v_max3_f32 v44, v44, v50, v51\n" \
+  "v_rsq_f32 v46, v46\n" \
+  "v_rsq_f32 v47, v47\n" \
+  "v_rsq_f32 v48, v48\n" \
+  "v_rsq_f32 v49, v49\n" \
+  "v_rsq_f32 v50, v50\n" \
+  "v_rsq_f32 v51, v51\n" \
+  "s_nop 0\n" \
+  "v_pk_mul_f32 v[116:117], v[116:117], v[2:3] op_sel:[0,0] op_sel_hi:[1,1] neg_lo:[0,0] neg_hi:[0,0]\n" \
+  "v_pk_mul_f32 v[118:119], v[118:119], v[8:9] op_sel:[0,0] op_sel_hi:[1,1] neg_lo:[0,0] neg_hi:[0,0]\n" \
+  "v_pk_mul_f32 v[70:71], v[70:71], v[46:47] op_sel:[0,0] op_sel_hi:[1,1] neg_lo:[0,0] neg_hi:[0,0]\n" \
+  "v_pk_mul_f32 v[228:229], v[228:229], v[46:47] op_sel:[0,0] op_sel_hi:[1,1] neg_lo:[0,0] neg_hi:[0,0]\n" \
+  "v_pk_mul_f32 v[116:117], v[116:117], v[46:47] op_sel:[0,0] op_sel_hi:[1,1] neg_lo:[0,0] neg_hi:[0,0]\n" \
+  "v_pk_mul_f32 v[118:119], v[118:119], v[46:47] op_sel:[0,0] op_sel_hi:[1,1] neg_lo:[0,0] neg_hi:[0,0]\n" \
+  "v_pk_mul_f32 v[70:71], v[70:71], v[46:47] op_sel:[0,0] op_sel_hi:[1,1] neg_lo:[0,0] neg_hi:[0,0]\n" \
+  "v_pk_mul_f32 v[120:121], v[120:121], v[4:5] op_sel:[0,0] op_sel_hi:[1,1] neg_lo:[0,0] neg_hi:[0,0]\n" \
+  "v_pk_mul_f32 v[122:123], v[122:123], v[10:11] op_sel:[0,0] op_sel_hi:[1,1] neg_lo:[0,0] neg_hi:[0,0]\n" \
+  "v_mul_f32 v218, v218, v34\n" \
+  "v_pk_mul_f32 v[72:73], v[72:73], v[48:49] op_sel:[0,0] op_sel_hi:[1,1] neg_lo:[0,0] neg_hi:[0,0]\n" \
+  "v_pk_mul_f32 v[230:231], v[230:231], v[48:49] op_sel:[0,0] op_sel_hi:[1,1] neg_lo:[0,0] neg_hi:[0,0]\n" \
+  "v_pk_mul_f32 v[120:121], v[120:121], v[48:49] op_sel:[0,0] op_sel_hi:[1,1] neg_lo:[0,0] neg_hi:[0,0]\n" \
+  "v_pk_mul_f32 v[122:123], v[122:123], v[48:49] op_sel:[0,0] op_sel_hi:[1,1] neg_lo:[0,0] neg_hi:[0,0]\n" \
+  "v_mul_f32 v218, v218, v49\n" \
+  "v_pk_mul_f32 v[72:73], v[72:73], v[48:49] op_sel:[0,0] op_sel_hi:[1,1] neg_lo:[0,0] neg_hi:[0,0]\n" \
+  "v_pk_mul_f32 v[124:125], v[124:125], v[6:7] op_sel:[0,0] op_sel_hi:[1,1] neg_lo:[0,0] neg_hi:[0,0]\n" \
+  "v_pk_mul_f32 v[126:127], v[126:127], v[12:13] op_sel:[0,0] op_sel_hi:[1,1] neg_lo:[0,0] neg_hi:[0,0]\n" \
+  "v_pk_mul_f32 v[128:129], v[128:129], v[32:33] op_sel:[0,0] op_sel_hi:[1,1] neg_lo:[0,0] neg_hi:[0,0]\n" \
+  "v_pk_mul_f32 v[74:75], v[74:75], v[50:51] op_sel:[0,0] op_sel_hi:[1,1] neg_lo:[0,0] neg_hi:[0,0]\n" \
+  "v_pk_mul_f32 v[232:233], v[232:233], v[50:51] op_sel:[0,0] op_sel_hi:[1,1] neg_lo:[0,0] neg_hi:[0,0]\n" \
+  "v_pk_mul_f32 v[124:125], v[124:125], v[50:51] op_sel:[0,0] op_sel_hi:[1,1] neg_lo:[0,0] neg_hi:[0,0]\n" \
+  "v_pk_mul_f32 v[126:127], v[126:127], v[50:51] op_sel:[0,0] op_sel_hi:[1,1] neg_lo:[0,0] neg_hi:[0,0]\n" \
+  "v_pk_mul_f32 v[128:129], v[128:129], v[50:51] op_sel:[0,0] op_sel_hi:[1,1] neg_lo:[0,0] neg_hi:[0,0]\n" \
+  "v_pk_mul_f32 v[74:75], v[74:75], v[50:51] op_sel:[0,0] op_sel_hi:[1,1] neg_lo:[0,0] neg_hi:[0,0]\n" \
+  "v_max3_f32 v46, |v76|, |v130|, |v132|\n" \
+  "v_max3_f32 v47, |v77|, |v131|, |v133|\n" \
+  "v_max3_f32 v48, |v78|, |v134|, |v136|\n" \
+  "v_max3_f32 v49, |v79|, |v135|, |v137|\n" \
+  "v_max3_f32 v50, |v80|, |v138|, |v140|\n" \
+  "v_max3_f32 v51, |v81|, |v139|, |v141|\n" \
+  "v_min3_f32 v43, v43, v46, v47\n" \
+  "v_max3_f32 v44, v44, v46, v47\n" \
+  "v_min3_f32 v43, v43, v48, v49\n" \
+  "v_max3_f32 v44, v44, v48, v49\n" \
+  "v_min3_f32 v43, v43, v50, v51\n" \
+  "v_max3_f32 v44, v44, v50, v51\n" \
+  "v_rsq_f32 v46, v46\n" \
+  "v_rsq_f32 v47, v47\n" \
+  "v_rsq_f32 v48, v48\n" \
+  "v_rsq_f32 v49, v49\n" \
+  "v_rsq_f32 v50, v50\n" \
+  "v_rsq_f32 v51, v51\n" \
+  "s_nop 0\n" \
+  "v_pk_mul_f32 v[130:131], v[130:131], v[8:9] op_sel:[0,0] op_sel_hi:[1,1] neg_lo:[0,0] neg_hi:[0,0]\n" \
+  "v_pk_mul_f32 v[132:133], v[132:133], v[14:15] op_sel:[0,0] op_sel_hi:[1,1] neg_lo:[0,0] neg_hi:[0,0]\n" \
+  "v_pk_mul_f32 v[76:77], v[76:77], v[46:47] op_sel:[0,0] op_sel_hi:[1,1] neg_lo:[0,0] neg_hi:[0,0]\n" \
+  "v_pk_mul_f32 v[234:235], v[234:235], v[46:47] op_sel:[0,0] op_sel_hi:[1,1] neg_lo:[0,0] neg_hi:[0,0]\n" \
+  "v_pk_mul_f32 v[130:131], v[130:131], v[46:47] op_sel:[0,0] op_sel_hi:[1,1] neg_lo:[0,0] neg_hi:[0,0]\n" \
+  "v_pk_mul_f32 v[132:133], v[132:133], v[46:47] op_sel:[0,0] op_sel_hi:[1,1] neg_lo:[0,0] neg_hi:[0,0]\n" \
+  "v_pk_mul_f32 v[76:77], v[76:77], v[46:47] op_sel:[0,0] op_sel_hi:[1,1] neg_lo:[0,0] neg_hi:[0,0]\n" \
+  "v_pk_mul_f32 v[134:135], v[134:135], v[10:11] op_sel:[0,0] op_sel_hi:[1,1] neg_lo:[0,0] neg_hi:[0,0]\n" \
+  "v_pk_mul_f32 v[136:137], v[136:137], v[16:17] op_sel:[0,0] op_sel_hi:[1,1] neg_lo:[0,0] neg_hi:[0,0]\n" \
+  "v_pk_mul_f32 v[78:79], v[78:79], v[48:49] op_sel:[0,0] op_sel_hi:[1,1] neg_lo:[0,0] neg_hi:[0,0]\n" \
+  "v_pk_mul_f32 v[236:237], v[236:237], v[48:49] op_sel:[0,0] op_sel_hi:[1,1] neg_lo:[0,0] neg_hi:[0,0]\n" \
+  "v_pk_mul_f32 v[134:135], v[134:135], v[48:49] op_sel:[0,0] op_sel_hi:[1,1] neg_lo:[0,0] neg_hi:[0,0]\n" \
+  "v_pk_mul_f32 v[136:137], v[136:137], v[48:49] op_sel:[0,0] op_sel_hi:[1,1] neg_lo:[0,0] neg_hi:[0,0]\n" \
+  "v_pk_mul_f32 v[78:79], v[78:79], v[48:49] op_sel:[0,0] op_sel_hi:[1,1] neg_lo:[0,0] neg_hi:[0,0]\n" \
+  "v_pk_mul_f32 v[138:139], v[138:139], v[12:13] op_sel:[0,0] op_sel_hi:[1,1] neg_lo:[0,0] neg_hi:[0,0]\n" \
+  "v_pk_mul_f32 v[140:141], v[140:141], v[18:19] op_sel:[0,0] op_sel_hi:[1,1] neg_lo:[0,0] neg_hi:[0,0]\n" \
+  "v_pk_mul_f32 v[80:81], v[80:81], v[50:51] op_sel:[0,0] op_sel_hi:[1,1] neg_lo:[0,0] neg_hi:[0,0]\n" \
+  "v_pk_mul_f32 v[238:239], v[238:239], v[50:51] op_sel:[0,0] op_sel_hi:[1,1] neg_lo:[0,0] neg_hi:[0,0]\n" \
+  "v_pk_mul_f32 v[138:139], v[138:139], v[50:51] op_sel:[0,0] op_sel_hi:[1,1] neg_lo:[0,0] neg_hi:[0,0]\n" \
+  "v_pk_mul_f32 v[140:141], v[140:141], v[50:51] op_sel:[0,0] op_sel_hi:[1,1] neg_lo:[0,0] neg_hi:[0,0]\n" \
+  "v_pk_mul_f32 v[80:81], v[80:81], v[50:51] op_sel:[0,0] op_sel_hi:[1,1] neg_lo:[0,0] neg_hi:[0,0]\n" \
+  "v_max_f32 v46, |v82|, |v142|\n" \
+  "v_max_f32 v47, |v83|, |v143|\n" \
+  "v_max_f32 v48, |v84|, |v144|\n" \
+  "v_max_f32 v49, |v85|, |v145|\n" \
+  "v_max_f32 v50, |v86|, |v146|\n" \
+  "v_max_f32 v51, |v87|, |v147|\n" \
+  "v_min3_f32 v43, v43, v46, v47\n" \
+  "v_max3_f32 v44, v44, v46, v47\n" \
+  "v_min3_f32 v43, v43, v48, v49\n" \
+  "v_max3_f32 v44, v44, v48, v49\n" \
+  "v_min3_f32 v43, v43, v50, v51\n" \
+  "v_max3_f32 v44, v44, v50, v51\n" \
+  "v_rsq_f32 v46, v46\n" \
+  "v_rsq_f32 v47, v47\n" \
+  "v_rsq_f32 v48, v48\n" \
+  "v_rsq_f32 v49, v49\n" \
+  "v_rsq_f32 v50, v50\n" \
+  "v_rsq_f32 v51, v51\n" \
+  "s_nop 0\n" \
+  "v_pk_mul_f32 v[142:143], v[142:143], v[14:15] op_sel:[0,0] op_sel_hi:[1,1] neg_lo:[0,0] neg_hi:[0,0]\n" \
+  "v_pk_mul_f32 v[82:83], v[82:83], v[46:47] op_sel:[0,0] op_sel_hi:[1,1] neg_lo:[0,0] neg_hi:[0,0]\n" \
+  "v_pk_mul_f32 v[240:241], v[240:241], v[46:47] op_sel:[0,0] op_sel_hi:[1,1] neg_lo:[0,0] neg_hi:[0,0]\n" \
+  "v_pk_mul_f32 v[142:143], v[142:143], v[46:47] op_sel:[0,0] op_sel_hi:[1,1] neg_lo:[0,0] neg_hi:[0,0]\n" \
+  "v_pk_mul_f32 v[82:83], v[82:83], v[46:47] op_sel:[0,0] op_sel_hi:[1,1] neg_lo:[0,0] neg_hi:[0,0]\n" \
+  "v_pk_mul_f32 v[144:145], v[144:145], v[16:17] op_sel:[0,0] op_sel_hi:[1,1] neg_lo:[0,0] neg_hi:[0,0]\n" \
+  "v_pk_mul_f32 v[84:85], v[84:85], v[48:49] op_sel:[0,0] op_sel_hi:[1,1] neg_lo:[0,0] neg_hi:[0,0]\n" \
+  "v_pk_mul_f32 v[242:243], v[242:243], v[48:49] op_sel:[0,0] op_sel_hi:[1,1] neg_lo:[0,0] neg_hi:[0,0]\n" \
+  "v_pk_mul_f32 v[144:145], v[144:145], v[48:49] op_sel:[0,0] op_sel_hi:[1,1] neg_lo:[0,0] neg_hi:[0,0]\n" \
+  "v_pk_mul_f32 v[84:85], v[84:85], v[48:49] op_sel:[0,0] op_sel_hi:[1,1] neg_lo:[0,0] neg_hi:[0,0]\n" \
+  "v_pk_mul_f32 v[146:147], v[146:147], v[18:19] op_sel:[0,0] op_sel_hi:[1,1] neg_lo:[0,0] neg_hi:[0,0]\n" \
+  "v_pk_mul_f32 v[86:87], v[86:87], v[50:51] op_sel:[0,0] op_sel_hi:[1,1] neg_lo:[0,0] neg_hi:[0,0]\n" \
+  "v_pk_mul_f32 v[244:245], v[244:245], v[50:51] op_sel:[0,0] op_sel_hi:[1,1] neg_lo:[0,0] neg_hi:[0,0]\n" \
+  "v_pk_mul_f32 v[146:147], v[146:147], v[50:51] op_sel:[0,0] op_sel_hi:[1,1] neg_lo:[0,0] neg_hi:[0,0]\n" \
+  "v_pk_mul_f32 v[86:87], v[86:87], v[50:51] op_sel:[0,0] op_sel_hi:[1,1] neg_lo:[0,0] neg_hi:[0,0]\n" \
+  "v_max3_f32 v46, |v88|, |v148|, |v150|\n" \
+  "v_max_f32 v46, v46, |v152|\n" \
+  "v_max3_f32 v47, |v89|, |v149|, |v151|\n" \
+  "v_max_f32 v47, v47, |v153|\n" \
+  "v_max3_f32 v48, |v90|, |v154|, |v156|\n" \
+  "v_max_f32 v48, v48, |v158|\n" \
+  "v_max3_f32 v49, |v91|, |v155|, |v157|\n" \
+  "v_max_f32 v49, v49, |v159|\n" \
+  "v_max3_f32 v50, |v92|, |v160|, |v162|\n" \
+  "v_max_f32 v50, v50, |v164|\n" \
+  "v_max3_f32 v51, |v93|, |v161|, |v163|\n" \
+  "v_max_f32 v51, v51, |v165|\n" \
+  "v_min3_f32 v43, v43, v46, v47\n" \
+  "v_max3_f32 v44, v44, v46, v47\n" \
+  "v_min3_f32 v43, v43, v48, v49\n" \
+  "v_max3_f32 v44, v44, v48, v49\n" \
+  "v_min3_f32 v43, v43, v50, v51\n" \
+  "v_max3_f32 v44, v44, v50, v51\n" \
+  "v_rsq_f32 v46, v46\n" \
+  "v_rsq_f32 v47, v47\n" \
+  "v_rsq_f32 v48, v48\n" \
+  "v_rsq_f32 v49, v49\n" \
+  "v_rsq_f32 v50, v50\n" \
+  "v_rsq_f32 v51, v51\n" \
+  "s_nop 0\n" \
+  "v_pk_mul_f32 v[148:149], v[148:149], v[2:3] op_sel:[0,0] op_sel_hi:[1,1] neg_lo:[0,0] neg_hi:[0,0]\n" \
+  "v_pk_mul_f32 v[150:151], v[150:151], v[20:21] op_sel:[0,0] op_sel_hi:[1,1] neg_lo:[0,0] neg_hi:[0,0]\n" \
+  "v_pk_mul_f32 v[152:153], v[152:153], v[26:27] op_sel:[0,0] op_sel_hi:[1,1] neg_lo:[0,0] neg_hi:[0,0]\n" \
+  "v_pk_mul_f32 v[88:89], v[88:89], v[46:47] op_sel:[0,0] op_sel_hi:[1,1] neg_lo:[0,0] neg_hi:[0,0]\n" \
+  "v_pk_mul_f32 v[246:247], v[246:247], v[46:47] op_sel:[0,0] op_sel_hi:[1,1] neg_lo:[0,0] neg_hi:[0,0]\n" \
+  "v_pk_mul_f32 v[148:149], v[148:149], v[46:47] op_sel:[0,0] op_sel_hi:[1,1] neg_lo:[0,0] neg_hi:[0,0]\n" \
+  "v_pk_mul_f32 v[150:151], v[150:151], v[46:47] op_sel:[0,0] op_sel_hi:[1,1] neg_lo:[0,0] neg_hi:[0,0]\n" \
+  "v_pk_mul_f32 v[152:153], v[152:153], v[46:47] op_sel:[0,0] op_sel_hi:[1,1] neg_lo:[0,0] neg_hi:[0,0]\n" \
+  "v_pk_mul_f32 v[88:89], v[88:89], v[46:47] op_sel:[0,0] op_sel_hi:[1,1] neg_lo:[0,0] neg_hi:[0,0]\n" \
+  "v_pk_mul_f32 v[154:155], v[154:155], v[4:5] op_sel:[0,0] op_sel_hi:[1,1] neg_lo:[0,0] neg_hi:[0,0]\n" \
+  "v_pk_mul_f32 v[156:157], v[156:157], v[22:23] op_sel:[0,0] op_sel_hi:[1,1] neg_lo:[0,0] neg_hi:[0,0]\n" \
+  "v_pk_mul_f32 v[158:159], v[158:159], v[28:29] op_sel:[0,0] op_sel_hi:[1,1] neg_lo:[0,0] neg_hi:[0,0]\n" \
+  "v_pk_mul_f32 v[90:91], v[90:91], v[48:49] op_sel:[0,0] op_sel_hi:[1,1] neg_lo:[0,0] neg_hi:[0,0]\n" \
+  "v_mul_f32 v248, v248, v48\n" \
+  "v_pk_mul_f32 v[154:155], v[154:155], v[48:49] op_sel:[0,0] op_sel_hi:[1,1] neg_lo:[0,0] neg_hi:[0,0]\n" \
+  "v_pk_mul_f32 v[156:157], v[156:157], v[48:49] op_sel:[0,0] op_sel_hi:[1,1] neg_lo:[0,0] neg_hi:[0,0]\n" \
+  "v_pk_mul_f32 v[158:159], v[158:159], v[48:49] op_sel:[0,0] op_sel_hi:[1,1] neg_lo:[0,0] neg_hi:[0,0]\n" \
+  "v_pk_mul_f32 v[90:91], v[90:91], v[48:49] op_sel:[0,0] op_sel_hi:[1,1] neg_lo:[0,0] neg_hi:[0,0]\n" \
+  "v_pk_mul_f32 v[160:161], v[160:161], v[6:7] op_sel:[0,0] op_sel_hi:[1,1] neg_lo:[0,0] neg_hi:[0,0]\n" \
+  "v_pk_mul_f32 v[162:163], v[162:163], v[24:25] op_sel:[0,0] op_sel_hi:[1,1] neg_lo:[0,0] neg_hi:[0,0]\n" \
+  "v_pk_mul_f32 v[164:165], v[164:165], v[30:31] op_sel:[0,0] op_sel_hi:[1,1] neg_lo:[0,0] neg_hi:[0,0]\n" \
+  "v_pk_mul_f32 v[92:93], v[92:93], v[50:51] op_sel:[0,0] op_sel_hi:[1,1] neg_lo:[0,0] neg_hi:[0,0]\n" \
+  "v_pk_mul_f32 v[160:161], v[160:161], v[50:51] op_sel:[0,0] op_sel_hi:[1,1] neg_lo:[0,0] neg_hi:[0,0]\n" \
+  "v_pk_mul_f32 v[162:163], v[162:163], v[50:51] op_sel:[0,0] op_sel_hi:[1,1] neg_lo:[0,0] neg_hi:[0,0]\n" \
+  "v_pk_mul_f32 v[164:165], v[164:165], v[50:51] op_sel:[0,0] op_sel_hi:[1,1] neg_lo:[0,0] neg_hi:[0,0]\n" \
+  "v_pk_mul_f32 v[92:93], v[92:93], v[50:51] op_sel:[0,0] op_sel_hi:[1,1] neg_lo:[0,0] neg_hi:[0,0]\n" \
+  "v_max3_f32 v46, |v94|, |v166|, |v168|\n" \
+  "v_max_f32 v46, v46, |v170|\n" \
+  "v_max3_f32 v47, |v95|, |v167|, |v169|\n" \
+  "v_max_f32 v47, v47, |v171|\n" \
+  "v_max3_f32 v48, |v96|, |v172|, |v174|\n" \
+  "v_max_f32 v48, v48, |v176|\n" \
+  "v_max3_f32 v49, |v97|, |v173|, |v175|\n" \
+  "v_max_f32 v49, v49, |v177|\n" \
+  "v_max3_f32 v50, |v98|, |v178|, |v180|\n" \
+  "v_max_f32 v50, v50, |v182|\n" \
+  "v_max3_f32 v51, |v99|, |v179|, |v181|\n" \
+  "v_max_f32 v51, v51, |v183|\n" \
+  "v_min3_f32 v43, v43, v46, v47\n" \
+  "v_max3_f32 v44, v44, v46, v47\n" \
+  "v_min3_f32 v43, v43, v48, v49\n" \
+  "v_max3_f32 v44, v44, v48, v49\n" \
+  "v_min3_f32 v43, v43, v50, v51\n" \
+  "v_max3_f32 v44, v44, v50, v51\n" \
+  "v_rsq_f32 v46, v46\n" \
+  "v_rsq_f32 v47, v47\n" \
+  "v_rsq_f32 v48, v48\n" \
+  "v_rsq_f32 v49, v49\n" \
+  "v_rsq_f32 v50, v50\n" \
+  "v_rsq_f32 v51, v51\n" \
+  "s_nop 0\n" \
+  "v_pk_mul_f32 v[166:167], v[166:167], v[8:9] op_sel:[0,0] op_sel_hi:[1,1] neg_lo:[0,0] neg_hi:[0,0]\n" \
+  "v_pk_mul_f32 v[168:169], v[168:169], v[26:27] op_sel:[0,0] op_sel_hi:[1,1] neg_lo:[0,0] neg_hi:[0,0]\n" \
+  "v_pk_mul_f32 v[170:171], v[170:171], v[32:33] op_sel:[0,0] op_sel_hi:[1,1] neg_lo:[0,0] neg_hi:[0,0]\n" \
+  "v_pk_mul_f32 v[94:95], v[94:95], v[46:47] op_sel:[0,0] op_sel_hi:[1,1] neg_lo:[0,0] neg_hi:[0,0]\n" \
+  "v_mul_f32 v249, v249, v46\n" \
+  "v_mul_f32 v250, v250, v47\n" \
+  "v_pk_mul_f32 v[166:167], v[166:167], v[46:47] op_sel:[0,0] op_sel_hi:[1,1] neg_lo:[0,0] neg_hi:[0,0]\n" \
+  "v_pk_mul_f32 v[168:169], v[168:169], v[46:47] op_sel:[0,0] op_sel_hi:[1,1] neg_lo:[0,0] neg_hi:[0,0]\n" \
+  "v_pk_mul_f32 v[170:171], v[170:171], v[46:47] op_sel:[0,0] op_sel_hi:[1,1] neg_lo:[0,0] neg_hi:[0,0]\n" \
+  "v_pk_mul_f32 v[94:95], v[94:95], v[46:47] op_sel:[0,0] op_sel_hi:[1,1] neg_lo:[0,0] neg_hi:[0,0]\n" \
+  "v_pk_mul_f32 v[172:173], v[172:173], v[10:11] op_sel:[0,0] op_sel_hi:[1,1] neg_lo:[0,0] neg_hi:[0,0]\n" \
+  "v_pk_mul_f32 v[174:175], v[174:175], v[28:29] op_sel:[0,0] op_sel_hi:[1,1] neg_lo:[0,0] neg_hi:[0,0]\n" \
+  "v_pk_mul_f32 v[176:177], v[176:177], v[34:35] op_sel:[0,0] op_sel_hi:[1,1] neg_lo:[0,0] neg_hi:[0,0]\n" \
+  "v_pk_mul_f32 v[96:97], v[96:97], v[48:49] op_sel:[0,0] op_sel_hi:[1,1] neg_lo:[0,0] neg_hi:[0,0]\n" \
+  "v_mul_f32 v251, v251, v48\n" \
+  "v_pk_mul_f32 v[172:173], v[172:173], v[48:49] op_sel:[0,0] op_sel_hi:[1,1] neg_lo:[0,0] neg_hi:[0,0]\n" \
+  "v_pk_mul_f32 v[174:175], v[174:175], v[48:49] op_sel:[0,0] op_sel_hi:[1,1] neg_lo:[0,0] neg_hi:[0,0]\n" \
+  "v_pk_mul_f32 v[176:177], v[176:177], v[48:49] op_sel:[0,0] op_sel_hi:[1,1] neg_lo:[0,0] neg_hi:[0,0]\n" \
+  "v_pk_mul_f32 v[96:97], v[96:97], v[48:49] op_sel:[0,0] op_sel_hi:[1,1] neg_lo:[0,0] neg_hi:[0,0]\n" \
+  "v_pk_mul_f32 v[178:179], v[178:179], v[12:13] op_sel:[0,0] op_sel_hi:[1,1] neg_lo:[0,0] neg_hi:[0,0]\n" \
+  "v_pk_mul_f32 v[180:181], v[180:181], v[30:31] op_sel:[0,0] op_sel_hi:[1,1] neg_lo:[0,0] neg_hi:[0,0]\n" \
+  "v_pk_mul_f32 v[182:183], v[182:183], v[36:37] op_sel:[0,0] op_sel_hi:[1,1] neg_lo:[0,0] neg_hi:[0,0]\n" \
+  "v_pk_mul_f32 v[98:99], v[98:99], v[50:51] op_sel:[0,0] op_sel_hi:[1,1] neg_lo:[0,0] neg_hi:[0,0]\n" \
+  "v_pk_mul_f32 v[178:179], v[178:179], v[50:51] op_sel:[0,0] op_sel_hi:[1,1] neg_lo:[0,0] neg_hi:[0,0]\n" \
+  "v_pk_mul_f32 v[180:181], v[180:181], v[50:51] op_sel:[0,0] op_sel_hi:[1,1] neg_lo:[0,0] neg_hi:[0,0]\n" \
+  "v_pk_mul_f32 v[182:183], v[182:183], v[50:51] op_sel:[0,0] op_sel_hi:[1,1] neg_lo:[0,0] neg_hi:[0,0]\n" \
+  "v_pk_mul_f32 v[98:99], v[98:99], v[50:51] op_sel:[0,0] op_sel_hi:[1,1] neg_lo:[0,0] neg_hi:[0,0]\n" \
+  "v_max3_f32 v46, |v100|, |v184|, |v186|\n" \
+  "v_max3_f32 v47, |v101|, |v185|, |v187|\n" \
+  "v_max3_f32 v48, |v102|, |v188|, |v190|\n" \
+  "v_max3_f32 v49, |v103|, |v189|, |v191|\n" \
+  "v_max3_f32 v50, |v104|, |v192|, |v194|\n" \
+  "v_max3_f32 v51, |v105|, |v193|, |v195|\n" \
+  "v_min3_f32 v43, v43, v46, v47\n" \
+  "v_max3_f32 v44, v44, v46, v47\n" \
+  "v_min3_f32 v43, v43, v48, v49\n" \
+  "v_max3_f32 v44, v44, v48, v49\n" \
+  "v_min3_f32 v43, v43, v50, v51\n" \
+  "v_max3_f32 v44, v44, v50, v51\n" \
+  "v_rsq_f32 v46, v46\n" \
+  "v_rsq_f32 v47, v47\n" \
+  "v_rsq_f32 v48, v48\n" \
+  "v_rsq_f32 v49, v49\n" \
+  "v_rsq_f32 v50, v50\n" \
+  "v_rsq_f32 v51, v51\n" \
+  "s_nop 0\n" \
+  "v_pk_mul_f32 v[184:185], v[184:185], v[14:15] op_sel:[0,0] op_sel_hi:[1,1] neg_lo:[0,0] neg_hi:[0,0]\n" \
+  "v_pk_mul_f32 v[186:187], v[186:187], v[32:33] op_sel:[0,0] op_sel_hi:[1,1] neg_lo:[0,0] neg_hi:[0,0]\n" \
+  "v_pk_mul_f32 v[100:101], v[100:101], v[46:47] op_sel:[0,0] op_sel_hi:[1,1] neg_lo:[0,0] neg_hi:[0,0]\n" \
+  "v_pk_mul_f32 v[252:253], v[252:253], v[46:47] op_sel:[0,0] op_sel_hi:[1,1] neg_lo:[0,0] neg_hi:[0,0]\n" \
+  "v_pk_mul_f32 v[184:185], v[184:185], v[46:47] op_sel:[0,0] op_sel_hi:[1,1] neg_lo:[0,0] neg_hi:[0,0]\n" \
+  "v_pk_mul_f32 v[186:187], v[186:187], v[46:47] op_sel:[0,0] op_sel_hi:[1,1] neg_lo:[0,0] neg_hi:[0,0]\n" \
+  "v_pk_mul_f32 v[100:101], v[100:101], v[46:47] op_sel:[0,0] op_sel_hi:[1,1] neg_lo:[0,0] neg_hi:[0,0]\n" \
+  "v_pk_mul_f32 v[188:189], v[188:189], v[16:17] op_sel:[0,0] op_sel_hi:[1,1] neg_lo:[0,0] neg_hi:[0,0]\n" \
+  "v_pk_mul_f32 v[190:191], v[190:191], v[34:35] op_sel:[0,0] op_sel_hi:[1,1] neg_lo:[0,0] neg_hi:[0,0]\n" \
+  "v_pk_mul_f32 v[102:103], v[102:103], v[48:49] op_sel:[0,0] op_sel_hi:[1,1] neg_lo:[0,0] neg_hi:[0,0]\n" \
+  "v_mul_f32 v254, v254, v48\n" \
+  "v_pk_mul_f32 v[188:189], v[188:189], v[48:49] op_sel:[0,0] op_sel_hi:[1,1] neg_lo:[0,0] neg_hi:[0,0]\n" \
+  "v_pk_mul_f32 v[190:191], v[190:191], v[48:49] op_sel:[0,0] op_sel_hi:[1,1] neg_lo:[0,0] neg_hi:[0,0]\n" \
+  "v_pk_mul_f32 v[102:103], v[102:103], v[48:49] op_sel:[0,0] op_sel_hi:[1,1] neg_lo:[0,0] neg_hi:[0,0]\n" \
+  "v_pk_mul_f32 v[192:193], v[192:193], v[18:19] op_sel:[0,0] op_sel_hi:[1,1] neg_lo:[0,0] neg_hi:[0,0]\n" \
+  "v_pk_mul_f32 v[194:195], v[194:195], v[36:37] op_sel:[0,0] op_sel_hi:[1,1] neg_lo:[0,0] neg_hi:[0,0]\n" \
+  "v_pk_mul_f32 v[104:105], v[104:105], v[50:51] op_sel:[0,0] op_sel_hi:[1,1] neg_lo:[0,0] neg_hi:[0,0]\n" \
+  "v_pk_mul_f32 v[192:193], v[192:193], v[50:51] op_sel:[0,0] op_sel_hi:[1,1] neg_lo:[0,0] neg_hi:[0,0]\n" \
+  "v_pk_mul_f32 v[194:195], v[194:195], v[50:51] op_sel:[0,0] op_sel_hi:[1,1] neg_lo:[0,0] neg_hi:[0,0]\n" \
+  "v_pk_mul_f32 v[104:105], v[104:105], v[50:51] op_sel:[0,0] op_sel_hi:[1,1] neg_lo:[0,0] neg_hi:[0,0]\n" \
+  "v_max3_f32 v46, |v106|, |v196|, |v197|\n" \
+  "v_max3_f32 v46, v46, |v198|, |v219|\n" \
+  "v_max3_f32 v47, |v107|, |v200|, |v201|\n" \
+  "v_max_f32 v47, v47, |v199|\n" \
+  "v_max3_f32 v48, |v108|, |v202|, |v203|\n" \
+  "v_max_f32 v48, v48, |v220|\n" \
+  "v_max3_f32 v49, |v109|, |v204|, |v205|\n" \
+  "v_max3_f32 v49, v49, |v221|, |v222|\n" \
+  "v_max3_f32 v50, |v110|, |v206|, |v207|\n" \
+  "v_max_f32 v50, v50, |v223|\n" \
+  "v_max3_f32 v51, |v111|, |v208|, |v209|\n" \
+  "v_max_f32 v51, v51, |v224|\n" \
+  "v_min3_f32 v43, v43, v46, v47\n" \
+  "v_max3_f32 v44, v44, v46, v47\n" \
+  "v_min3_f32 v43, v43, v48, v49\n" \
+  "v_max3_f32 v44, v44, v48, v49\n" \
+  "v_min3_f32 v43, v43, v50, v51\n" \
+  "v_max3_f32 v44, v44, v50, v51\n" \
+  "v_rsq_f32 v46, v46\n" \
+  "v_rsq_f32 v47, v47\n" \
+  "v_rsq_f32 v48, v48\n" \
+  "v_rsq_f32 v49, v49\n" \
+  "v_rsq_f32 v50, v50\n" \
+  "v_rsq_f32 v51, v51\n" \
+  "s_nop 0\n" \
+  "v_pk_mul_f32 v[196:197], v[196:197], v[20:21] op_sel:[0,0] op_sel_hi:[1,1] neg_lo:[0,0] neg_hi:[0,0]\n" \
+  "v_pk_mul_f32 v[198:199], v[198:199], v[22:23] op_sel:[0,0] op_sel_hi:[1,1] neg_lo:[0,0] neg_hi:[0,0]\n" \
+  "v_pk_mul_f32 v[200:201], v[200:201], v[24:25] op_sel:[0,0] op_sel_hi:[1,1] neg_lo:[0,0] neg_hi:[0,0]\n" \
+  "v_mul_f32 v219, v219, v38\n" \
+  "v_pk_mul_f32 v[106:107], v[106:107], v[46:47] op_sel:[0,0] op_sel_hi:[1,1] neg_lo:[0,0] neg_hi:[0,0]\n" \
+  "v_pk_mul_f32 v[196:197], v[196:197], v[46:47] op_sel:[0,0] op_sel_hi:[1,0] neg_lo:[0,0] neg_hi:[0,0]\n" \
+  "v_pk_mul_f32 v[198:199], v[198:199], v[46:47] op_sel:[0,0] op_sel_hi:[1,1] neg_lo:[0,0] neg_hi:[0,0]\n" \
+  "v_pk_mul_f32 v[200:201], v[200:201], v[46:47] op_sel:[0,1] op_sel_hi:[1,1] neg_lo:[0,0] neg_hi:[0,0]\n" \
+  "v_mul_f32 v219, v219, v46\n" \
+  "v_pk_mul_f32 v[106:107], v[106:107], v[46:47] op_sel:[0,0] op_sel_hi:[1,1] neg_lo:[0,0] neg_hi:[0,0]\n" \
+  "v_pk_mul_f32 v[202:203], v[202:203], v[24:25] op_sel:[0,0] op_sel_hi:[1,1] neg_lo:[0,0] neg_hi:[0,0]\n" \
+  "v_pk_mul_f32 v[204:205], v[204:205], v[26:27] op_sel:[0,0] op_sel_hi:[1,1] neg_lo:[0,0] neg_hi:[0,0]\n" \
+  "v_mul_f32 v220, v220, v23\n" \
+  "v_mul_f32 v221, v221, v28\n" \
+  "v_mul_f32 v222, v222, v39\n" \
+  "v_pk_mul_f32 v[108:109], v[108:109], v[48:49] op_sel:[0,0] op_sel_hi:[1,1] neg_lo:[0,0] neg_hi:[0,0]\n" \
+  "v_pk_mul_f32 v[202:203], v[202:203], v[48:49] op_sel:[0,0] op_sel_hi:[1,0] neg_lo:[0,0] neg_hi:[0,0]\n" \
+  "v_pk_mul_f32 v[204:205], v[204:205], v[48:49] op_sel:[0,1] op_sel_hi:[1,1] neg_lo:[0,0] neg_hi:[0,0]\n" \
+  "v_mul_f32 v220, v220, v48\n" \
+  "v_mul_f32 v221, v221, v49\n" \
+  "v_mul_f32 v222, v222, v49\n" \
+  "v_pk_mul_f32 v[108:109], v[108:109], v[48:49] op_sel:[0,0] op_sel_hi:[1,1] neg_lo:[0,0] neg_hi:[0,0]\n" \
+  "v_pk_mul_f32 v[206:207], v[206:207], v[30:31] op_sel:[0,0] op_sel_hi:[1,1] neg_lo:[0,0] neg_hi:[0,0]\n" \
+  "v_pk_mul_f32 v[208:209], v[208:209], v[30:31] op_sel:[0,0] op_sel_hi:[1,1] neg_lo:[0,0] neg_hi:[0,0]\n" \
+  "v_mul_f32 v223, v223, v29\n" \
+  "v_mul_f32 v224, v224, v29\n" \
+  "v_pk_mul_f32 v[110:111], v[110:111], v[50:51] op_sel:[0,0] op_sel_hi:[1,1] neg_lo:[0,0] neg_hi:[0,0]\n" \
+  "v_pk_mul_f32 v[206:207], v[206:207], v[50:51] op_sel:[0,0] op_sel_hi:[1,0] neg_lo:[0,0] neg_hi:[0,0]\n" \
+  "v_pk_mul_f32 v[208:209], v[208:209], v[50:51] op_sel:[0,1] op_sel_hi:[1,1] neg_lo:[0,0] neg_hi:[0,0]\n" \
+  "v_mul_f32 v223, v223, v50\n" \
+  "v_mul_f32 v224, v224, v51\n" \
+  "v_pk_mul_f32 v[110:111], v[110:111], v[50:51] op_sel:[0,0] op_sel_hi:[1,1] neg_lo:[0,0] neg_hi:[0,0]\n" \
+  "v_max3_f32 v46, |v112|, |v210|, |v211|\n" \
+  "v_max3_f32 v46, v46, |v212|, |v225|\n" \
+  "v_max3_f32 v47, |v113|, |v214|, |v215|\n" \
+  "v_max_f32 v47, v47, |v213|\n" \
+  "v_max3_f32 v48, |v114|, |v216|, |v217|\n" \
+  "v_max_f32 v48, v48, |v226|\n" \
+  "v_mov_b32 v49, 1.0\n" \
+  "v_min3_f32 v43, v43, v46, v47\n" \
+  "v_max3_f32 v44, v44, v46, v47\n" \
+  "v_min_f32 v43, v43, v48\n" \
+  "v_max_f32 v44, v44, v48\n" \
+  "v_rsq_f32 v46, v46\n" \
+  "v_rsq_f32 v47, v47\n" \
+  "v_rsq_f32 v48, v48\n" \
+  "s_nop 0\n" \
+  "v_pk_mul_f32 v[210:211], v[210:211], v[32:33] op_sel:[0,0] op_sel_hi:[1,1] neg_lo:[0,0] neg_hi:[0,0]\n" \
+  "v_pk_mul_f32 v[212:213], v[212:213], v[34:35] op_sel:[0,0] op_sel_hi:[1,1] neg_lo:[0,0] neg_hi:[0,0]\n" \
+  "v_pk_mul_f32 v[214:215], v[214:215], v[36:37] op_sel:[0,0] op_sel_hi:[1,1] neg_lo:[0,0] neg_hi:[0,0]\n" \
+  "v_mul_f32 v225, v225, v40\n" \
+  "v_pk_mul_f32 v[112:113], v[112:113], v[46:47] op_sel:[0,0] op_sel_hi:[1,1] neg_lo:[0,0] neg_hi:[0,0]\n" \
+  "v_pk_mul_f32 v[210:211], v[210:211], v[46:47] op_sel:[0,0] op_sel_hi:[1,0] neg_lo:[0,0] neg_hi:[0,0]\n" \
+  "v_pk_mul_f32 v[212:213], v[212:213], v[46:47] op_sel:[0,0] op_sel_hi:[1,1] neg_lo:[0,0] neg_hi:[0,0]\n" \
+  "v_pk_mul_f32 v[214:215], v[214:215], v[46:47] op_sel:[0,1] op_sel_hi:[1,1] neg_lo:[0,0] neg_hi:[0,0]\n" \
+  "v_mul_f32 v225, v225, v46\n" \
+  "v_pk_mul_f32 v[112:113], v[112:113], v[46:47] op_sel:[0,0] op_sel_hi:[1,1] neg_lo:[0,0] neg_hi:[0,0]\n" \
+  "v_pk_mul_f32 v[216:217], v[216:217], v[36:37] op_sel:[0,0] op_sel_hi:[1,1] neg_lo:[0,0] neg_hi:[0,0]\n" \
+  "v_mul_f32 v226, v226, v35\n" \
+  "v_mul_f32 v114, v114, v48\n" \
+  "v_pk_mul_f32 v[216:217], v[216:217], v[48:49] op_sel:[0,0] op_sel_hi:[1,0] neg_lo:[0,0] neg_hi:[0,0]\n" \
+  "v_mul_f32 v226, v226, v48\n" \
+  "v_mul_f32 v114, v114, v48\n" \
+  "v_pk_add_f32 v[46:47], v[70:71], v[72:73] op_sel:[0,0] op_sel_hi:[1,1] neg_lo:[0,0] neg_hi:[0,0]\n" \
+  "v_pk_add_f32 v[46:47], v[46:47], v[74:75] op_sel:[0,0] op_sel_hi:[1,1] neg_lo:[0,0] neg_hi:[0,0]\n" \
+  "v_pk_add_f32 v[46:47], v[46:47], v[76:77] op_sel:[0,0] op_sel_hi:[1,1] neg_lo:[0,0] neg_hi:[0,0]\n" \
+  "v_pk_add_f32 v[46:47], v[46:47], v[78:79] op_sel:[0,0] op_sel_hi:[1,1] neg_lo:[0,0] neg_hi:[0,0]\n" \
+  "v_pk_add_f32 v[46:47], v[46:47], v[80:81] op_sel:[0,0] op_sel_hi:[1,1] neg_lo:[0,0] neg_hi:[0,0]\n" \
+  "v_pk_add_f32 v[46:47], v[46:47], v[82:83] op_sel:[0,0] op_sel_hi:[1,1] neg_lo:[0,0] neg_hi:[0,0]\n" \
+  "v_pk_add_f32 v[46:47], v[46:47], v[84:85] op_sel:[0,0] op_sel_hi:[1,1] neg_lo:[0,0] neg_hi:[0,0]\n" \
+  "v_pk_add_f32 v[46:47], v[46:47], v[86:87] op_sel:[0,0] op_sel_hi:[1,1] neg_lo:[0,0] neg_hi:[0,0]\n" \
+  "v_pk_add_f32 v[46:47], v[46:47], v[88:89] op_sel:[0,0] op_sel_hi:[1,1] neg_lo:[0,0] neg_hi:[0,0]\n" \
+  "v_pk_add_f32 v[46:47], v[46:47], v[90:91] op_sel:[0,0] op_sel_hi:[1,1] neg_lo:[0,0] neg_hi:[0,0]\n" \
+  "v_pk_add_f32 v[46:47], v[46:47], v[92:93] op_sel:[0,0] op_sel_hi:[1,1] neg_lo:[0,0] neg_hi:[0,0]\n" \
+  "v_pk_add_f32 v[46:47], v[46:47], v[94:95] op_sel:[0,0] op_sel_hi:[1,1] neg_lo:[0,0] neg_hi:[0,0]\n" \
+  "v_pk_add_f32 v[46:47], v[46:47], v[96:97] op_sel:[0,0] op_sel_hi:[1,1] neg_lo:[0,0] neg_hi:[0,0]\n" \
+  "v_pk_add_f32 v[46:47], v[46:47], v[98:99] op_sel:[0,0] op_sel_hi:[1,1] neg_lo:[0,0] neg_hi:[0,0]\n" \
+  "v_pk_add_f32 v[46:47], v[46:47], v[100:101] op_sel:[0,0] op_sel_hi:[1,1] neg_lo:[0,0] neg_hi:[0,0]\n" \
+  "v_pk_add_f32 v[46:47], v[46:47], v[102:103] op_sel:[0,0] op_sel_hi:[1,1] neg_lo:[0,0] neg_hi:[0,0]\n" \
+  "v_pk_add_f32 v[46:47], v[46:47], v[104:105] op_sel:[0,0] op_sel_hi:[1,1] neg_lo:[0,0] neg_hi:[0,0]\n" \
+  "v_pk_add_f32 v[46:47], v[46:47], v[106:107] op_sel:[0,0] op_sel_hi:[1,1] neg_lo:[0,0] neg_hi:[0,0]\n" \
+  "v_pk_add_f32 v[46:47], v[46:47], v[108:109] op_sel:[0,0] op_sel_hi:[1,1] neg_lo:[0,0] neg_hi:[0,0]\n" \
+  "v_pk_add_f32 v[46:47], v[46:47], v[110:111] op_sel:[0,0] op_sel_hi:[1,1] neg_lo:[0,0] neg_hi:[0,0]\n" \
+  "v_pk_add_f32 v[46:47], v[46:47], v[112:113] op_sel:[0,0] op_sel_hi:[1,1] neg_lo:[0,0] neg_hi:[0,0]\n" \
+  "v_pk_add_f32 v[46:47], v[46:47], v[114:115] op_sel:[0,0] op_sel_hi:[1,1] neg_lo:[0,0] neg_hi:[0,0]\n" \
+  "v_max3_f32 v45, |v228|, |v229|, |v230|\n" \
+  "v_max3_f32 v45, v45, |v231|, |v232|\n" \
+  "v_max3_f32 v45, v45, |v233|, |v234|\n" \
+  "v_max3_f32 v45, v45, |v235|, |v236|\n" \
+  "v_max3_f32 v45, v45, |v237|, |v238|\n" \
+  "v_max3_f32 v45, v45, |v239|, |v240|\n" \
+  "v_max3_f32 v45, v45, |v241|, |v242|\n" \
+  "v_max3_f32 v45, v45, |v243|, |v244|\n" \
+  "v_max3_f32 v45, v45, |v245|, |v246|\n" \
+  "v_max3_f32 v45, v45, |v247|, |v248|\n" \
+  "v_max3_f32 v45, v45, |v249|, |v250|\n" \
+  "v_max3_f32 v45, v45, |v251|, |v252|\n" \
+  "v_max3_f32 v45, v45, |v253|, |v254|\n" \
+  "v_add_f32 v46, v46, v47\n" \
+  "v_mul_f32 v46, s18, v46\n" \
+  "v_cmp_lt_f32 vcc, s16, v45\n" \
+  "v_cndmask_b32 v45, 1.0, v45, vcc\n" \
+  "v_min_f32 v45, s17, v45\n" \
+  "v_max_f32 v46, v46, v45\n" \
+  "v_cmp_lt_f32 vcc, s16, v46\n" \
+  "v_cndmask_b32 v46, 1.0, v46, vcc\n" \
+  "v_min_f32 v46, s17, v46\n" \
+  "v_rcp_f32 v48, v46\n" \
+  "s_nop 0\n" \
+  "v_fma_f32 v49, -v46, v48, 1.0\n" \
+  "v_fma_f32 v48, v49, v48, v48\n" \
+  "v_pk_mul_f32 v[70:71], v[70:71], v[48:49] op_sel:[0,0] op_sel_hi:[1,0] neg_lo:[0,0] neg_hi:[0,0]\n" \
+  "v_pk_mul_f32 v[72:73], v[72:73], v[48:49] op_sel:[0,0] op_sel_hi:[1,0] neg_lo:[0,0] neg_hi:[0,0]\n" \
+  "v_pk_mul_f32 v[74:75], v[74:75], v[48:49] op_sel:[0,0] op_sel_hi:[1,0] neg_lo:[0,0] neg_hi:[0,0]\n" \
+  "v_pk_mul_f32 v[76:77], v[76:77], v[48:49] op_sel:[0,0] op_sel_hi:[1,0] neg_lo:[0,0] neg_hi:[0,0]\n" \
+  "v_pk_mul_f32 v[78:79], v[78:79], v[48:49] op_sel:[0,0] op_sel_hi:[1,0] neg_lo:[0,0] neg_hi:[0,0]\n" \
+  "v_pk_mul_f32 v[80:81], v[80:81], v[48:49] op_sel:[0,0] op_sel_hi:[1,0] neg_lo:[0,0] neg_hi:[0,0]\n" \
+  "v_pk_mul_f32 v[82:83], v[82:83], v[48:49] op_sel:[0,0] op_sel_hi:[1,0] neg_lo:[0,0] neg_hi:[0,0]\n" \
+  "v_pk_mul_f32 v[84:85], v[84:85], v[48:49] op_sel:[0,0] op_sel_hi:[1,0] neg_lo:[0,0] neg_hi:[0,0]\n" \
+  "v_pk_mul_f32 v[86:87], v[86:87], v[48:49] op_sel:[0,0] op_sel_hi:[1,0] neg_lo:[0,0] neg_hi:[0,0]\n" \
+  "v_pk_mul_f32 v[88:89], v[88:89], v[48:49] op_sel:[0,0] op_sel_hi:[1,0] neg_lo:[0,0] neg_hi:[0,0]\n" \
+  "v_pk_mul_f32 v[90:91], v[90:91], v[48:49] op_sel:[0,0] op_sel_hi:[1,0] neg_lo:[0,0] neg_hi:[0,0]\n" \
+  "v_pk_mul_f32 v[92:93], v[92:93], v[48:49] op_sel:[0,0] op_sel_hi:[1,0] neg_lo:[0,0] neg_hi:[0,0]\n" \
+  "v_pk_mul_f32 v[94:95], v[94:95], v[48:49] op_sel:[0,0] op_sel_hi:[1,0] neg_lo:[0,0] neg_hi:[0,0]\n" \
+  "v_pk_mul_f32 v[96:97], v[96:97], v[48:49] op_sel:[0,0] op_sel_hi:[1,0] neg_lo:[0,0] neg_hi:[0,0]\n" \
+  "v_pk_mul_f32 v[98:99], v[98:99], v[48:49] op_sel:[0,0] op_sel_hi:[1,0] neg_lo:[0,0] neg_hi:[0,0]\n" \
+  "v_pk_mul_f32 v[100:101], v[100:101], v[48:49] op_sel:[0,0] op_sel_hi:[1,0] neg_lo:[0,0] neg_hi:[0,0]\n" \
+  "v_pk_mul_f32 v[102:103], v[102:103], v[48:49] op_sel:[0,0] op_sel_hi:[1,0] neg_lo:[0,0] neg_hi:[0,0]\n" \
+  "v_pk_mul_f32 v[104:105], v[104:105], v[48:49] op_sel:[0,0] op_sel_hi:[1,0] neg_lo:[0,0] neg_hi:[0,0]\n" \
+  "v_pk_mul_f32 v[106:107], v[106:107], v[48:49] op_sel:[0,0] op_sel_hi:[1,0] neg_lo:[0,0] neg_hi:[0,0]\n" \
+  "v_pk_mul_f32 v[108:109], v[108:109], v[48:49] op_sel:[0,0] op_sel_hi:[1,0] neg_lo:[0,0] neg_hi:[0,0]\n" \
+  "v_pk_mul_f32 v[110:111], v[110:111], v[48:49] op_sel:[0,0] op_sel_hi:[1,0] neg_lo:[0,0] neg_hi:[0,0]\n" \
+  "v_pk_mul_f32 v[112:113], v[112:113], v[48:49] op_sel:[0,0] op_sel_hi:[1,0] neg_lo:[0,0] neg_hi:[0,0]\n" \
+  "v_pk_mul_f32 v[114:115], v[114:115], v[48:49] op_sel:[0,0] op_sel_hi:[1,0] neg_lo:[0,0] neg_hi:[0,0]\n" \
+  "v_pk_mul_f32 v[228:229], v[228:229], v[48:49] op_sel:[0,0] op_sel_hi:[1,0] neg_lo:[0,0] neg_hi:[0,0]\n" \
+  "v_pk_mul_f32 v[230:231], v[230:231], v[48:49] op_sel:[0,0] op_sel_hi:[1,0] neg_lo:[0,0] neg_hi:[0,0]\n" \
+  "v_pk_mul_f32 v[232:233], v[232:233], v[48:49] op_sel:[0,0] op_sel_hi:[1,0] neg_lo:[0,0] neg_hi:[0,0]\n" \
+  "v_pk_mul_f32 v[234:235], v[234:235], v[48:49] op_sel:[0,0] op_sel_hi:[1,0] neg_lo:[0,0] neg_hi:[0,0]\n" \
+  "v_pk_mul_f32 v[236:237], v[236:237], v[48:49] op_sel:[0,0] op_sel_hi:[1,0] neg_lo:[0,0] neg_hi:[0,0]\n" \
+  "v_pk_mul_f32 v[238:239], v[238:239], v[48:49] op_sel:[0,0] op_sel_hi:[1,0] neg_lo:[0,0] neg_hi:[0,0]\n" \
+  "v_pk_mul_f32 v[240:241], v[240:241], v[48:49] op_sel:[0,0] op_sel_hi:[1,0] neg_lo:[0,0] neg_hi:[0,0]\n" \
+  "v_pk_mul_f32 v[242:243], v[242:243], v[48:49] op_sel:[0,0] op_sel_hi:[1,0] neg_lo:[0,0] neg_hi:[0,0]\n" \
+  "v_pk_mul_f32 v[244:245], v[244:245], v[48:49] op_sel:[0,0] op_sel_hi:[1,0] neg_lo:[0,0] neg_hi:[0,0]\n" \
+  "v_pk_mul_f32 v[246:247], v[246:247], v[48:49] op_sel:[0,0] op_sel_hi:[1,0] neg_lo:[0,0] neg_hi:[0,0]\n" \
+  "v_pk_mul_f32 v[248:249], v[248:249], v[48:49] op_sel:[0,0] op_sel_hi:[1,0] neg_lo:[0,0] neg_hi:[0,0]\n" \
+  "v_pk_mul_f32 v[250:251], v[250:251], v[48:49] op_sel:[0,0] op_sel_hi:[1,0] neg_lo:[0,0] neg_hi:[0,0]\n" \
+  "v_pk_mul_f32 v[252:253], v[252:253], v[48:49] op_sel:[0,0] op_sel_hi:[1,0] neg_lo:[0,0] neg_hi:[0,0]\n" \
+  "v_pk_mul_f32 v[254:255], v[254:255], v[48:49] op_sel:[0,0] op_sel_hi:[1,0] neg_lo:[0,0] neg_hi:[0,0]\n" \
+  "v_mul_f32 v42, v42, v48\n" \
+  "s_sub_i32 s15, s15, 1\n" \
+  "s_cmp_gt_i32 s15, 0\n" \
+  "s_cbranch_scc1 503b\n" \
+  "v_cmp_lt_f32_e64 s[30:31], s16, v43\n" \
+  "v_cmp_ge_f32_e64 s[32:33], s17, v44\n" \
+  "s_and_b64 s[30:31], s[30:31], s[32:33]\n" \
+  "s_andn2_b64 s[30:31], exec, s[30:31]\n" \
+  "s_cbranch_scc0 505f\n" \
+  "s_mov_b32 s14, 1\n" \
+  "s_waitcnt vmcnt(0) lgkmcnt(0)\n" \
+  "s_branch 501b\n" \
+  "504:\n" \
   "s_cmp_gt_i32 s15, 0\n" \
   "s_cbranch_scc1 28b\n" \
+  "505:\n" \
   "v_rcp_f32 v43, v42\n" \
   "s_nop 0\n" \
   "v_fma_f32 v44, -v42, v43, 1.0\n" \
diff --git a/robobee3d_amd/isasim.py b/robobee3d_amd/isasim.py
--- a/robobee3d_amd/isasim.py
+++ b/robobee3d_amd/isasim.py
@@ -116,6 +116,7 @@
         self.max_exec, self.quad, self.log = max_exec, quad or {}, log
         self.nexec = 0
         self.sections = {}
+        self.hits = None
         self.pend = {"vmcnt": [], "lgkmcnt": []}
         self.labels = {}
         for k, t in enumerate(ins):
@@ -310,6 +311,8 @@
                     return
                 self.nexec += 1
                 assert self.nexec < self.max_exec, "runaway program"
+                if self.hits is not None:
+                    self.hits[self.pc] += 1
                 if m == "s_waitcnt":
                     self.wait(t)
                 elif m == "s_barrier":
@@ -503,13 +506,7 @@
 
 
 def _nanless(red):
-    def f(a, b, c):
-        out = np.empty_like(a)
-        for ln in range(len(a)):
-            vals = [x for x in (a[ln], b[ln], c[ln]) if x == x]
-            out[ln] = red(vals) if vals else f32(np.nan)
-        return out
-    return f
+    return lambda a, b, c: red(red(a, b), c)
 
 
 def _f64op(op):
@@ -646,8 +643,8 @@
     "v_max_f32": _f32op(_fmax),
     "v_max_f32_dpp": _f32op(_fmax, True),
     "v_min_f32": _f32op(_fmin),
-    "v_max3_f32": _f32op(_nanless(max)),
-    "v_min3_f32": _f32op(_nanless(min)),
+    "v_max3_f32": _f32op(_nanless(np.fmax)),
+    "v_min3_f32": _f32op(_nanless(np.fmin)),
     "v_med3_f32": _f32op(lambda a, b, c: np.sort(np.stack([a, b, c]), 0)[1]),
     "v_rcp_f32": _f32op(lambda a: f32(1.0) / a),
     "v_rsq_f32": _f32op(lambda a: (1.0 / np.sqrt(a.astype(f64))).astype(f32)),
```

Measured after the change: 546.5 million (median of 6 runs). 1.01x the previous value.
